# JoeHEZHAO/Optical-Flow-Guided-Feature-Pytorch

Measured on AMD Instinct MI355X. Metric: OFF-forward clips/sec (7-seg 224x224), higher is better.
Workload: dtype f32 (split-fp32: every fp32 operand as three bf16 planes = the fp32 value exactly, six exact plane products on the bf16 MFMA pipe, f32 accumulate); 1 GPU; RGB_OFF forward, batch=64 clips/GPU x 7 segments, nine 224x224-geometry feature maps; global_batch=64, segments=7, parallelism=clip-shard x1, slice_mode=reference_flat

## Files before the change

### include/offk.h

```cpp
#ifndef OFFK_H_
#define OFFK_H_

#include <stddef.h>
#include <stdint.h>

#ifdef __cplusplus
extern "C" {
#endif

#define OFFK_ABI_VERSION 10
#define OFFK_NUM_SITES 9

enum offk_status {
  OFFK_OK = 0,
  OFFK_ERR_INVALID = -1,
  OFFK_ERR_HIP = -2,
  OFFK_ERR_MISSING_WEIGHT = -3,
  OFFK_ERR_UNKNOWN_KEY = -4,
  OFFK_ERR_NO_DEVICE = -5
};

enum offk_variant {
  OFFK_VARIANT_RGB_LEARNED_DW = 0,
  OFFK_VARIANT_DIAG_SOBEL = 1
};
enum offk_slice_mode {
  OFFK_SLICE_REFERENCE_FLAT = 0,
  OFFK_SLICE_PER_CLIP = 1
};
enum offk_consensus {
  OFFK_CONSENSUS_NONE = 0,
  OFFK_CONSENSUS_AVG = 1
};
enum offk_feat_layout {
  OFFK_FEAT_NCHW = 0,
  OFFK_FEAT_NHWC = 1
};

enum offk_precision {
  OFFK_PRECISION_FP32 = 0,
  OFFK_PRECISION_F32SPLIT = 2
};

typedef struct offk_config {
  int32_t batch;
  int32_t length;
  int32_t variant;
  int32_t slice_mode;
  int32_t consensus;
  int32_t num_classes;
  int32_t feat_layout;
  int32_t device;
  int32_t precision;
} offk_config;

typedef struct offk_handle offk_handle;

int offk_abi_version(void);

const char* offk_last_error(const offk_handle* h);

int offk_create(const offk_config* cfg, offk_handle** out);
int offk_destroy(offk_handle* h);

int offk_set_weight(offk_handle* h, const char* key, const float* data, const int64_t* shape, int ndim);
int offk_bind_weight(offk_handle* h, const char* key, const float* device_data, const int64_t* shape, int ndim);
int offk_missing_weights(const offk_handle* h, char* buf, size_t buflen);

size_t offk_workspace_bytes(const offk_handle* h);

int offk_forward(offk_handle* h, void* stream, const float* const feats[OFFK_NUM_SITES],
                 float* out7, float* out14, float* out28, void* workspace);

typedef struct offk_feat_parts {
  int32_t n_parts;
  int32_t channels[4];
  const float* data[4];
} offk_feat_parts;
int offk_forward_parts(offk_handle* h, void* stream, const offk_feat_parts parts[OFFK_NUM_SITES],
                       float* out7, float* out14, float* out28, void* workspace);

enum offk_feat_dtype { OFFK_FEAT_F32 = 0, OFFK_FEAT_BF16 = 1, OFFK_FEAT_F16 = 2 };
int offk_forward_typed(offk_handle* h, void* stream, int feat_dtype, const void* const feats[OFFK_NUM_SITES],
                       float* out7, float* out14, float* out28, void* workspace);
int offk_forward_parts_typed(offk_handle* h, void* stream, int feat_dtype, const offk_feat_parts parts[OFFK_NUM_SITES],
                             float* out7, float* out14, float* out28, void* workspace);

int offk_forward_cl(offk_handle* h, void* stream, int feat_dtype, const void* const feats[OFFK_NUM_SITES],
                    float* out7, float* out14, float* out28, void* workspace);
int offk_forward_parts_cl(offk_handle* h, void* stream, int feat_dtype, const offk_feat_parts parts[OFFK_NUM_SITES],
                          float* out7, float* out14, float* out28, void* workspace);

int offk_workspace_region(const offk_handle* h, const char* name, size_t* offset_bytes, size_t* nbytes);

#define OFFK_NUM_STAGES 6
int offk_set_profiling(offk_handle* h, int enable);
int offk_stage_times(offk_handle* h, double ms[OFFK_NUM_STAGES], int64_t calls[OFFK_NUM_STAGES], int reset);
int offk_launch_times(offk_handle* h, char* names, size_t names_len, double* ms, int64_t* calls, int max_entries, int reset);


int offk_pw_reduce(offk_handle* h, void* stream, int site, const float* feat, float* G, float* D);

int offk_sobel_tdiff(offk_handle* h, void* stream, int site, const float* G, const float* D,
                     float* M, int m_cstride, int m_coff, int algo);

int offk_sobel_tdiff_all(offk_handle* h, void* stream, void* workspace, int algo);

int offk_off_units(offk_handle* h, void* stream, const float* const feats[OFFK_NUM_SITES], void* workspace);
int offk_off_units_fused(offk_handle* h, void* stream, const float* const feats[OFFK_NUM_SITES], void* workspace);
int offk_off_units_fused_typed(offk_handle* h, void* stream, int feat_dtype, const void* const feats[OFFK_NUM_SITES],
                               void* workspace);
int offk_off_units_fused_cl(offk_handle* h, void* stream, int feat_dtype, const void* const feats[OFFK_NUM_SITES],
                            void* workspace);

enum offk_conv_flags { OFFK_CONV_RELU_IN = 1, OFFK_CONV_RELU_PRE = 2, OFFK_CONV_RELU_POST = 4,
                        };
int offk_conv2d(void* stream, const float* x, int x_cstride, int x_coff, int n_img, int H, int W, int Ci,
                const float* w, const float* bias, int Co, int KH, int KW, int stride, int pad,
                const float* res, int res_cstride, int res_coff, int flags,
                float* y, int y_cstride, int y_coff);
int offk_conv2d_ex(void* stream, const float* x, int x_cstride, int x_coff, int n_img, int H, int W, int Ci,
                   const float* w, const float* bias, int Co, int KH, int KW, int stride, int pad,
                   const float* res, int res_cstride, int res_coff, int flags,
                   float* y, int y_cstride, int y_coff, int tile_cfg, int splitk, float* partial, size_t partial_floats,
                   int precision);
int offk_pack_conv_weight(void* stream, const float* w_oihw, int Co, int Ci, int KH, int KW, float* w_packed);
int offk_set_conv_plan(offk_handle* h, const char* conv_key, int tile_cfg, int splitk);

int offk_bottleneck_chain14(void* stream, const float* x, int x_cstride, int x_coff, int n_img, int Cin, int relu_in,
                            const float* w1, const float* b1, const float* w2_packed, const float* b2,
                            const float* w3, const float* b3, int K3,
                            const float* res, int res_cstride, int res_coff, float* y, int y_cstride, int y_coff);
int offk_bottleneck_chain14_split(void* stream, const float* x, int x_cstride, int x_coff, int n_img, int Cin, int relu_in,
                                  const float* w1, const float* b1, const float* w2_packed, const float* b2,
                                  const float* w3, const float* b3, const float* branch_w, const float* branch_b,
                                  const float* res, int res_cstride, int res_coff, float* y, int y_cstride, int y_coff,
                                  void* scratch, size_t scratch_bytes);
int offk_winograd_conv3x3(void* stream, const float* x, int x_cstride, int x_coff, int n_img, int Ci,
                          const float* w_packed, const float* bias, int Co,
                          const float* res, int res_cstride, int res_coff, int flags,
                          float* y, int y_cstride, int y_coff, float* scratch, size_t scratch_floats, float* pool_part);

int offk_winograd_conv5x5s2(void* stream, const float* x, int x_cstride, int x_coff, int n_img, int Ci,
                            const float* w_packed, const float* bias, int Co,
                            const float* res, int res_cstride, int res_coff, int flags,
                            float* y, int y_cstride, int y_coff, float* scratch, size_t scratch_floats);

int offk_winograd_conv7x7s2(void* stream, const float* x, int x_cstride, int x_coff, int n_img, int Ci,
                            const float* w_packed, const float* bias, int Co, int flags,
                            float* y, int y_cstride, int y_coff, float* scratch, size_t scratch_floats);

int offk_winograd_between(void* stream, const float* M, const float* bias_in, int phases_in, int n_img, int Cin,
                          float* x, int x_cstride, int x_coff, const float* w1, const float* b1, int Cmid, float* V);
int offk_winograd_between_ex(void* stream, const float* M, const float* bias_in, int phases_in, int n_img, int Cin, float* x,
                             int x_cstride, int x_coff, const float* w1, const float* b1, int Cmid, float* V, int precision,
                             void* scratch, size_t scratch_bytes);

int offk_batched_gemm_nt(void* stream, const float* x, const float* w, float* y, int batch, int M, int K, int Co, int precision,
                         void* scratch, size_t scratch_bytes);

int offk_head(void* stream, const float* x, int x_cstride, int x_coff, int n_img, int H, int W, int C,
              int maxpool, const float* fc_w, const float* fc_b, int num_classes, float* out);

int offk_segment_consensus(void* stream, const float* x, int B, int T, int C, float* out);

int offk_score_fusion(void* stream, const float* const* scores, const float* weights, int n_sets, int videos,
                      int crops, int classes, float* fused, int32_t* pred);

typedef struct offk_grad_view {
  const float* data;
  int32_t cstride;
  int32_t coff;
} offk_grad_view;

size_t offk_train_workspace_bytes(const offk_handle* h);

// ... 38 lines not shown
```

### optical-flow-guided-feature-pytorch_amd/_lib.py

```python
import ctypes
import os

HERE = os.path.dirname(os.path.abspath(__file__))
LIB_PATH = os.environ.get("OFFK_LIB") or os.path.join(HERE, "liboffk.so")
NUM_SITES = 9
NUM_STAGES = 6
STAGE_NAMES = ("pw_reduce", "sobel_tdiff", "fusion_28", "fusion_14", "fusion_7", "heads")

CONV_RELU_IN, CONV_RELU_PRE, CONV_RELU_POST = 1, 2, 4
PRECISION_FP32, PRECISION_F32SPLIT = 0, 2
PRECISIONS = {"fp32": 0, "f32split": 2}
FEAT_F32, FEAT_BF16, FEAT_F16 = 0, 1, 2


class OffkError(RuntimeError):
    pass


class OffkConfig(ctypes.Structure):
    _fields_ = [("batch", ctypes.c_int32), ("length", ctypes.c_int32), ("variant", ctypes.c_int32),
                ("slice_mode", ctypes.c_int32), ("consensus", ctypes.c_int32),
                ("num_classes", ctypes.c_int32), ("feat_layout", ctypes.c_int32),
                ("device", ctypes.c_int32), ("precision", ctypes.c_int32)]


class OffkFeatParts(ctypes.Structure):
    _fields_ = [("n_parts", ctypes.c_int32), ("channels", ctypes.c_int32 * 4), ("data", ctypes.c_void_p * 4)]


class OffkGradView(ctypes.Structure):
    _fields_ = [("data", ctypes.c_void_p), ("cstride", ctypes.c_int32), ("coff", ctypes.c_int32)]


_c = ctypes
_P = ctypes.c_void_p
_F = ctypes.c_void_p
_I = ctypes.c_int

SIGNATURES = {
    "offk_abi_version": (_I, []),
    "offk_last_error": (_c.c_char_p, [_P]),
    "offk_create": (_I, [_c.POINTER(OffkConfig), _c.POINTER(_P)]),
    "offk_destroy": (_I, [_P]),
    "offk_set_weight": (_I, [_P, _c.c_char_p, _F, _c.POINTER(_c.c_int64), _I]),
    "offk_bind_weight": (_I, [_P, _c.c_char_p, _F, _c.POINTER(_c.c_int64), _I]),
    "offk_missing_weights": (_I, [_P, _c.c_char_p, _c.c_size_t]),
    "offk_workspace_bytes": (_c.c_size_t, [_P]),
    "offk_forward": (_I, [_P, _P, _c.POINTER(_F), _F, _F, _F, _P]),
    "offk_forward_parts": (_I, [_P, _P, _c.POINTER(OffkFeatParts), _F, _F, _F, _P]),
    "offk_forward_typed": (_I, [_P, _P, _I, _c.POINTER(_P), _F, _F, _F, _P]),
    "offk_forward_parts_typed": (_I, [_P, _P, _I, _c.POINTER(OffkFeatParts), _F, _F, _F, _P]),
    "offk_forward_cl": (_I, [_P, _P, _I, _c.POINTER(_P), _F, _F, _F, _P]),
    "offk_forward_parts_cl": (_I, [_P, _P, _I, _c.POINTER(OffkFeatParts), _F, _F, _F, _P]),
    "offk_workspace_region": (_I, [_P, _c.c_char_p, _c.POINTER(_c.c_size_t), _c.POINTER(_c.c_size_t)]),
    "offk_set_profiling": (_I, [_P, _I]),
    "offk_stage_times": (_I, [_P, _c.POINTER(_c.c_double), _c.POINTER(_c.c_int64), _I]),
    "offk_launch_times": (_I, [_P, _c.c_char_p, _c.c_size_t, _c.POINTER(_c.c_double), _c.POINTER(_c.c_int64), _I, _I]),
    "offk_pw_reduce": (_I, [_P, _P, _I, _F, _F, _F]),
    "offk_sobel_tdiff": (_I, [_P, _P, _I, _F, _F, _F, _I, _I, _I]),
    "offk_sobel_tdiff_all": (_I, [_P, _P, _P, _I]),
    "offk_off_units": (_I, [_P, _P, _c.POINTER(_F), _P]),
    "offk_off_units_fused": (_I, [_P, _P, _c.POINTER(_F), _P]),
    "offk_off_units_fused_typed": (_I, [_P, _P, _I, _c.POINTER(_P), _P]),
    "offk_off_units_fused_cl": (_I, [_P, _P, _I, _c.POINTER(_P), _P]),
    "offk_conv2d": (_I, [_P, _F, _I, _I, _I, _I, _I, _I, _F, _F, _I, _I, _I, _I, _I, _F, _I, _I, _I, _F, _I, _I]),
    "offk_conv2d_ex": (_I, [_P, _F, _I, _I, _I, _I, _I, _I, _F, _F, _I, _I, _I, _I, _I, _F, _I, _I, _I, _F, _I, _I,
                            _I, _I, _F, _c.c_size_t, _I]),
    "offk_bottleneck_chain14": (_I, [_P, _F, _I, _I, _I, _I, _I, _F, _F, _F, _F, _F, _F, _I, _F, _I, _I, _F, _I, _I]),
    "offk_bottleneck_chain14_split": (_I, [_P, _F, _I, _I, _I, _I, _I, _F, _F, _F, _F, _F, _F, _F, _F, _F, _I, _I, _F, _I, _I, _P, ctypes.c_size_t]),
    "offk_winograd_conv3x3": (_I, [_P, _F, _I, _I, _I, _I, _F, _F, _I, _F, _I, _I, _I, _F, _I, _I, _F, _c.c_size_t, _F]),
    "offk_winograd_conv5x5s2": (_I, [_P, _F, _I, _I, _I, _I, _F, _F, _I, _F, _I, _I, _I, _F, _I, _I, _F, _c.c_size_t]),
    "offk_winograd_conv7x7s2": (_I, [_P, _F, _I, _I, _I, _I, _F, _F, _I, _I, _F, _I, _I, _F, _c.c_size_t]),
    "offk_winograd_between": (_I, [_P, _F, _F, _I, _I, _I, _F, _I, _I, _F, _F, _I, _F]),
    "offk_winograd_between_ex": (_I, [_P, _F, _F, _I, _I, _I, _F, _I, _I, _F, _F, _I, _F, _I, _P, ctypes.c_size_t]),
    "offk_batched_gemm_nt": (_I, [_P, _F, _F, _F, _I, _I, _I, _I, _I, _P, _c.c_size_t]),
    "offk_pack_conv_weight": (_I, [_P, _F, _I, _I, _I, _I, _F]),
    "offk_set_conv_plan": (_I, [_P, _c.c_char_p, _I, _I]),
    "offk_head": (_I, [_P, _F, _I, _I, _I, _I, _I, _I, _I, _F, _F, _I, _F]),
    "offk_segment_consensus": (_I, [_P, _F, _I, _I, _I, _F]),
    "offk_score_fusion": (_I, [_P, _c.POINTER(_F), _c.POINTER(_c.c_float), _I, _I, _I, _I, _F, _F]),
    "offk_train_workspace_bytes": (_c.c_size_t, [_P]),
    "offk_off_units_train": (_I, [_P, _P, _c.POINTER(_F), _P, _c.c_uint64, _c.c_double]),
    "offk_unit_grad_floats": (_c.c_size_t, [_P]),
    "offk_unit_grad_slot": (_I, [_P, _c.c_char_p, _c.POINTER(_c.c_size_t), _c.POINTER(_c.c_size_t)]),
    "offk_off_units_backward": (_I, [_P, _P, _c.POINTER(_F), _c.POINTER(OffkGradView), _P, _c.c_uint64, _c.c_double, _F, _I]),
    "offk_pw_reduce_typed": (_I, [_P, _P, _I, _I, _P, _F, _F]),
    "offk_off_units_typed": (_I, [_P, _P, _I, _c.POINTER(_P), _P]),
    "offk_off_units_train_typed": (_I, [_P, _P, _I, _c.POINTER(_P), _P, _c.c_uint64, _c.c_double]),
    "offk_off_units_backward_typed": (_I, [_P, _P, _I, _c.POINTER(_P), _c.POINTER(OffkGradView), _P, _c.c_uint64, _c.c_double, _F, _I]),
    "offk_pw_reduce_cl": (_I, [_P, _P, _I, _I, _P, _F, _F]),
    "offk_off_units_cl": (_I, [_P, _P, _I, _c.POINTER(_P), _P]),
    "offk_off_units_train_cl": (_I, [_P, _P, _I, _c.POINTER(_P), _P, _c.c_uint64, _c.c_double]),
    "offk_off_units_backward_cl": (_I, [_P, _P, _I, _c.POINTER(_P), _c.POINTER(OffkGradView), _P, _c.c_uint64, _c.c_double, _F, _I]),
    "offk_segment_consensus_backward": (_I, [_P, _F, _I, _I, _I, _F]),
    "offk_nchw_to_nhwc": (_I, [_P, _F, _I, _I, _I, _F]),
    "offk_nhwc_to_nchw": (_I, [_P, _F, _I, _I, _I, _I, _I, _F]),
}

_lib = None


def load():
    global _lib
    if _lib is not None:
        return _lib
    import torch
    if not os.path.exists(LIB_PATH):
        raise OffkError("liboffk.so not built: run `python -c 'import __graft_entry__ as g; g.build()'` "
                        "(or optical-flow-guided-feature-pytorch_amd/build.py); there is no fallback path")
    lib = ctypes.CDLL(LIB_PATH)
    for name, (res, args) in SIGNATURES.items():
        fn = getattr(lib, name)
        fn.restype = res
        fn.argtypes = args
    if lib.offk_abi_version() != 10:
        raise OffkError("liboffk.so ABI version mismatch")
    _lib = lib
    return lib


def check(rc, handle=None):
    if rc != 0:
        msg = load().offk_last_error(handle)
        raise OffkError("liboffk error %d: %s" % (rc, msg.decode() if msg else "?"))
```

### optical-flow-guided-feature-pytorch_amd/csrc/heads.hip

```cpp
#include "offk_common.h"
#include "offk_internal.h"

#include <mutex>
#include <set>
#include <utility>

namespace offk {

hipError_t lds_attr_once(const void* kernel, int bytes) {
  static std::mutex mu;
  static std::set<std::pair<const void*, int>> done;
  int dev = 0;
  hipError_t e = hipGetDevice(&dev);
  if (e != hipSuccess) return e;
  std::lock_guard<std::mutex> lock(mu);
  if (done.count({kernel, dev})) return hipSuccess;
  e = hipFuncSetAttribute(kernel, hipFuncAttributeMaxDynamicSharedMemorySize, bytes);
  if (e == hipSuccess) done.insert({kernel, dev});
  return e;
}

constexpr int HEAD_MAX_C = 1024;

__device__ __forceinline__ float4 add4(float4 a, float4 b) { return make_float4(a.x + b.x, a.y + b.y, a.z + b.z, a.w + b.w); }
// ... 209 lines not shown
  float pw[4];
#pragma unroll
  for (int j = 0; j < 4; ++j) {
    const int sl = min(s_lo + j, s_hi);
    const int slot = (sl * 32) / hw == img ? 0 : 1;
    ps[j] = tiles ? part + ((size_t)img * 4 + j) * C + 4 * kq : part + ((size_t)sl * 2 + slot) * C + 4 * kq;
    pw[j] = tiles || s_lo + j <= s_hi ? 1.f : 0.f;
  }
  const int per = ((C / kFcWaves + 63) / 64) * 64;
  const int kbeg = wave * per, kend = min(C, kbeg + per);
  const float* w0 = fw + (size_t)min(cls0 + li, ncls - 1) * C + 4 * kq;
  const float* w1 = fw + (size_t)min(cls0 + 16 + li, ncls - 1) * C + 4 * kq;
  fcx4 acc0 = {0.f, 0.f, 0.f, 0.f}, acc1 = {0.f, 0.f, 0.f, 0.f};
  for (int kb = kbeg; kb < kend; kb += 64) {
    fcx4 xr[4][4], a0[4], a1[4];
#pragma unroll
    for (int u = 0; u < 4; ++u) {
#pragma unroll
      for (int j = 0; j < 4; ++j) xr[u][j] = *reinterpret_cast<const fcx4*>(ps[j] + kb + 16 * u);
      a0[u] = *reinterpret_cast<const fcx4*>(w0 + kb + 16 * u);
      a1[u] = *reinterpret_cast<const fcx4*>(w1 + kb + 16 * u);
    }
#pragma unroll
    for (int u = 0; u < 4; ++u) {
      const fcx4 x = ((xr[u][0] * pw[0] + xr[u][1] * pw[1]) + xr[u][2] * pw[2]) + xr[u][3] * pw[3];
      acc0 = __builtin_amdgcn_mfma_f32_16x16x4f32(a0[u].x, x.x, acc0, 0, 0, 0);
      acc1 = __builtin_amdgcn_mfma_f32_16x16x4f32(a1[u].x, x.x, acc1, 0, 0, 0);
      acc0 = __builtin_amdgcn_mfma_f32_16x16x4f32(a0[u].y, x.y, acc0, 0, 0, 0);
      acc1 = __builtin_amdgcn_mfma_f32_16x16x4f32(a1[u].y, x.y, acc1, 0, 0, 0);
      acc0 = __builtin_amdgcn_mfma_f32_16x16x4f32(a0[u].z, x.z, acc0, 0, 0, 0);
      acc1 = __builtin_amdgcn_mfma_f32_16x16x4f32(a1[u].z, x.z, acc1, 0, 0, 0);
      acc0 = __builtin_amdgcn_mfma_f32_16x16x4f32(a0[u].w, x.w, acc0, 0, 0, 0);
      acc1 = __builtin_amdgcn_mfma_f32_16x16x4f32(a1[u].w, x.w, acc1, 0, 0, 0);
    }
  }
  red[wave][0][lane] = acc0;
  red[wave][1][lane] = acc1;
  __syncthreads();
  if (wave < 2) {
    fcx4 v = red[0][wave][lane];
#pragma unroll
    for (int w = 1; w < kFcWaves; ++w) v += red[w][wave][lane];
    const int gi = blockIdx.x * 16 + li, c = cls0 + 16 * wave + 4 * kq;
    const float inv = 1.f / (float)hw;
    if (gi < n_img) {
#pragma unroll
      for (int j = 0; j < 4; ++j)
        if (c + j < ncls) out[(size_t)gi * ncls + c + j] = v[j] * inv + fb[c + j];
    }
  }
}
__global__ __launch_bounds__(64 * kFcWaves) void fc_pooled_kernel(const float* __restrict__ part, int hw, int tiles, int n_img, int C,
                                                                  const float* __restrict__ fw, const float* __restrict__ fb, int ncls,
                                                                  float* __restrict__ out) {
  fc_pooled_body(part, hw, tiles, n_img, C, fw, fb, ncls, out);
}
__global__ __launch_bounds__(64 * kFcWaves) void fc_pooled_multi_kernel(FcPooledJobs j) {
  const FcPooledJob& h = j.job[blockIdx.z];
  fc_pooled_body(h.part, h.hw, h.tiles, j.n_img, h.C, h.fw, h.fb, j.ncls, h.out);
}
hipError_t fc_pooled_multi_launch(const FcPooledJobs& j, hipStream_t st) {
  if (j.njobs < 1 || j.njobs > 3 || j.n_img <= 0 || j.ncls <= 0) return hipErrorInvalidValue;
  for (int i = 0; i < j.njobs; ++i)
    if (j.job[i].C % 64 || j.job[i].hw < 32) return hipErrorInvalidValue;
  hipLaunchKernelGGL(fc_pooled_multi_kernel, dim3((j.n_img + 15) / 16, (j.ncls + 31) / 32, j.njobs), dim3(64 * kFcWaves), 0, st, j);
  return hipGetLastError();
}
hipError_t fc_pooled_launch(const float* part, int hw, int tiles, int n_img, int C, const float* fw, const float* fb, int ncls, float* out,
                            hipStream_t st) {
  if (C % 64 || hw < 32 || n_img <= 0 || ncls <= 0) return hipErrorInvalidValue;
  hipLaunchKernelGGL(fc_pooled_kernel, dim3((n_img + 15) / 16, (ncls + 31) / 32), dim3(64 * kFcWaves), 0, st, part, hw, tiles, n_img, C, fw, fb, ncls, out);
  return hipGetLastError();
}

__global__ void vec_add_kernel(const float* __restrict__ a, const float* __restrict__ b, float* __restrict__ o, int n) {
  int i = blockIdx.x * blockDim.x + threadIdx.x;
  if (i < n) o[i] = a[i] + b[i];
}
hipError_t vec_add_launch(const float* a, const float* b, float* o, int n, hipStream_t st) {
  hipLaunchKernelGGL(vec_add_kernel, dim3((n + 255) / 256), dim3(256), 0, st, a, b, o, n);
  return hipGetLastError();
}

__global__ void consensus_kernel(const float* __restrict__ x, int T, int C, float* __restrict__ out) {
  const int b = blockIdx.x;
  for (int c = threadIdx.x; c < C; c += blockDim.x) {
    float s = 0.f;
    for (int t = 0; t < T; ++t) s += x[((size_t)b * T + t) * C + c];
    out[(size_t)b * C + c] = s / (float)T;
  }
}
__global__ void consensus_multi_kernel(const float* x0, const float* x1, const float* x2, int T, int C, float* o0, float* o1, float* o2) {
  const float* const x = blockIdx.y == 0 ? x0 : blockIdx.y == 1 ? x1 : x2;
  float* const out = blockIdx.y == 0 ? o0 : blockIdx.y == 1 ? o1 : o2;
  const int b = blockIdx.x;
  for (int c = threadIdx.x; c < C; c += blockDim.x) {
    float s = 0.f;
    for (int t = 0; t < T; ++t) s += x[((size_t)b * T + t) * C + c];
    out[(size_t)b * C + c] = s / (float)T;
  }
}
hipError_t consensus_multi_launch(const float* const x[3], float* const out[3], int nheads, int B, int T, int C, hipStream_t st) {
  if (nheads < 1 || nheads > 3) return hipErrorInvalidValue;
  hipLaunchKernelGGL(consensus_multi_kernel, dim3(B, nheads), dim3(128), 0, st, x[0], x[1], x[2], T, C, out[0], out[1], out[2]);
  return hipGetLastError();
}
hipError_t consensus_launch(const float* x, int B, int T, int C, float* out, hipStream_t st) {
  hipLaunchKernelGGL(consensus_kernel, dim3(B), dim3(128), 0, st, x, T, C, out);
  return hipGetLastError();
}

constexpr int SF_MAX_SETS = 8;
struct ScoreFusionArgs { const float* s[SF_MAX_SETS]; float w[SF_MAX_SETS]; int n, crops, classes; float* fused; int* pred; };
__global__ __launch_bounds__(256) void score_fusion_kernel(ScoreFusionArgs a) {
  __shared__ float best_v[256];
  __shared__ int best_i[256];
  const int v = blockIdx.x, tid = threadIdx.x;
  float bv = -INFINITY;
  int bi = 0x7fffffff;
  for (int c = tid; c < a.classes; c += 256) {
    float acc = 0.f;
#pragma unroll
    for (int i = 0; i < SF_MAX_SETS; ++i)
      if (i < a.n) {
        const float* p = a.s[i] + ((size_t)v * a.crops) * a.classes + c;
        float m = 0.f;
        for (int k = 0; k < a.crops; ++k) m += p[(size_t)k * a.classes];
        acc += a.w[i] * (m / (float)a.crops);
      }
    a.fused[(size_t)v * a.classes + c] = acc;
    if (acc > bv) { bv = acc; bi = c; }
  }
  if (!a.pred) return;
  best_v[tid] = bv; best_i[tid] = bi;
  __syncthreads();
  for (int s = 128; s > 0; s >>= 1) {
    if (tid < s) {
      const float ov = best_v[tid + s];
      const int oi = best_i[tid + s];
      if (ov > best_v[tid] || (ov == best_v[tid] && oi < best_i[tid])) { best_v[tid] = ov; best_i[tid] = oi; }
    }
    __syncthreads();
  }
  if (tid == 0) a.pred[v] = best_i[0];
}
hipError_t score_fusion_launch(const float* const* scores, const float* weights, int n, int videos, int crops, int classes,
                               float* fused, int* pred, hipStream_t st) {
  if (n < 1 || n > SF_MAX_SETS) return hipErrorInvalidValue;
  ScoreFusionArgs a;
  for (int i = 0; i < SF_MAX_SETS; ++i) { a.s[i] = i < n ? scores[i] : nullptr; a.w[i] = i < n ? weights[i] : 0.f; }
  a.n = n; a.crops = crops; a.classes = classes; a.fused = fused; a.pred = pred;
  hipLaunchKernelGGL(score_fusion_kernel, dim3(videos), dim3(256), 0, st, a);
  return hipGetLastError();
}

__global__ __launch_bounds__(256) void nchw_to_nhwc_kernel(const float* __restrict__ src, int C, int HW, float* __restrict__ dst) {
  __shared__ float t[32][33];
  const int n = blockIdx.z, c0 = blockIdx.y * 32, q0 = blockIdx.x * 32;
  const int tx = threadIdx.x & 31, ty = threadIdx.x >> 5;
  for (int r = ty; r < 32; r += 8) {
    int c = c0 + r, q = q0 + tx;
    t[r][tx] = (c < C && q < HW) ? src[((size_t)n * C + c) * HW + q] : 0.f;
  }
  __syncthreads();
  for (int r = ty; r < 32; r += 8) {
    int q = q0 + r, c = c0 + tx;
// ... 32 lines not shown
```

### optical-flow-guided-feature-pytorch_amd/csrc/offk_api.hip

```cpp
#include "../../include/offk.h"

#include <algorithm>
#include <cmath>
#include <cstdio>
#include <cstdlib>
#include <cstring>
#include <map>
#include <string>
#include <vector>

#include "offk_internal.h"

using namespace offk;

typedef const void* const* MapPtrs;

static bool path_switch(const char* name, int* min_p = nullptr) {
  const char* e = getenv(name);
  if (e && min_p && atoi(e) > 1) *min_p = atoi(e);
  return !(e && *e == '0');
}

static ConvDesc conv_desc(const float* x, int x_cs, int x_coff, int n_img, int H, int W, int Ci, const float* w, const float* bias, int Co, int KH,
                          int KW, int stride, int pad, const float* res, int res_cs, int res_coff, int flags, float* y, int y_cs, int y_coff,
// ... 17 lines not shown
      a.g_x[gi] = grp[gi].v_off; a.g_w[gi] = grp[gi].u_off; a.g_y[gi] = grp[gi].m_off;
    }
    a.w_planes = U_planes;
    if (U_planes && wino_gemm_split_supported(a)) return wino_gemm_split_launch(a, s);
    if (persistent && wino_gemm_supported(a)) return wino_gemm_launch(a, s);
  }
  const int K0 = grp[0].kmul * Ci;
  ConvDesc d = conv_desc(V, K0, 0, rows, 1, 1, K0, U, nullptr, Co, 1, 1, 1, 0, nullptr, 0, 0, 0, M, Co, 0, 3, 1);
#ifdef OFFK_TUNING_KNOBS
  { const char* e = getenv("OFFK_WINO_CFG"); if (e && (Co % 128 == 0 || atoi(e) == 1 || atoi(e) == 2)) d.tile_cfg = atoi(e); }
#endif
  d.batch = npoints; d.x_bstride = (long long)rows * K0; d.w_bstride = (long long)Co * K0; d.y_bstride = (long long)rows * Co;
  if (ngrp > 1) {
    d.ngroups = ngrp;
    for (int gi = 0; gi < ngrp; ++gi) {
      d.g_batch[gi] = grp[gi].batch; d.g_Ci[gi] = grp[gi].kmul * Ci;
      d.g_x[gi] = grp[gi].v_off; d.g_w[gi] = grp[gi].u_off; d.g_y[gi] = grp[gi].m_off;
    }
  }
  return conv2d_launch(d, s, why);
}
static bool wino_gemm_stage_default() {
  static const bool on = path_switch("OFFK_WINO_GEMM");
  return on;
}

namespace {

struct SiteSpec { const char* name; int C, H; };
const SiteSpec kSites[kNumSites] = {{"3a", 256, 28}, {"3b", 320, 28}, {"3c", 576, 14}, {"4a", 576, 14}, {"4b", 576, 14},
                                    {"4c", 608, 14}, {"4d", 608, 14}, {"5a", 1024, 7}, {"5b", 1024, 7}};
const int kPwOrder[kNumSites] = {7, 8, 5, 6, 2, 3, 4, 1, 0};
const int kSiteFusion[kNumSites] = {0, 0, 1, 1, 1, 1, 1, 2, 2};
const int kSiteCoff[kNumSites] = {0, 160, 0, 160, 320, 480, 640, 0, 160};
const int kFusionC[3] = {320, 1056, 832};

struct ConvSpec { const char* key; int Co, Ci, K, stride, pad; };
enum ConvId {
  C_T28, C1_28A, C2_28A, C3_28A, CB_28A, C1_28B, C2_28B, C3_28B, C1_28C, C2_28C, C3_28C,
  C_T14, C1_14A, C2_14A, C3_14A, CE_14A, C1_14B, C2_14B, C3_14B,
  C_T7, C1_7, C2_7, C3_7, CB_7, kNumConvs
};
const ConvSpec kConvs[kNumConvs] = {
    {"motion_conv_trans_28", 64, 320, 7, 2, 3},      {"motion_conv1_trans_28a", 64, 64, 1, 1, 0},
    {"motion_conv2_trans_28a", 64, 64, 3, 1, 1},     {"motion_conv3_trans_28a", 256, 64, 1, 1, 0},
    {"motion_conv_branch_28a", 256, 64, 1, 1, 0},    {"motion_conv1_trans_28b", 64, 256, 1, 1, 0},
    {"motion_conv2_trans_28b", 64, 64, 3, 1, 1},     {"motion_conv3_trans_28b", 256, 64, 1, 1, 0},
    {"motion_conv1_trans_28c", 64, 256, 1, 1, 0},    {"motion_conv2_trans_28c", 64, 64, 3, 1, 1},
    {"motion_conv3_trans_28c", 256, 64, 1, 1, 0},    {"motion_conv_trans_14", 128, 1056, 5, 2, 2},
    {"motion_conv1_trans_14a", 128, 128, 1, 1, 0},   {"motion_conv2_trans_14a", 128, 128, 3, 1, 1},
    {"motion_conv3_trans_14a", 512, 128, 1, 1, 0},   {"motion_conv_expand_trans_14a", 512, 128, 1, 1, 0},
    {"motion_conv1_trans_14b", 128, 512, 1, 1, 0},   {"motion_conv2_trans_14b", 128, 128, 3, 1, 1},
    {"motion_conv3_trans_14b", 512, 128, 3, 1, 1},   {"motion_conv_trans", 256, 832, 3, 1, 1},
    {"motion_conv1_trans", 256, 256, 1, 1, 0},       {"motion_conv2_trans", 256, 256, 3, 1, 1},
    {"motion_conv3_trans", 1024, 256, 1, 1, 0},      {"motion_conv_branch_trans", 1024, 256, 1, 1, 0}};
struct MergedSpec { const char* name; int main_id, branch_id; };
const MergedSpec kMerged[3] = {{"merged_28a", C3_28A, CB_28A}, {"merged_14a", C3_14A, CE_14A}, {"merged_7", C3_7, CB_7}};
const int kTunedP240[kNumConvs][2] = {
    {3, 2}, {-1, 0}, {-1, 0}, {-1, 0}, {-1, 0}, {-1, 0}, {-1, 0}, {-1, 0}, {-1, 0}, {-1, 0}, {-1, 0},
    {4, 4}, {-1, 0}, {-1, 0}, {-1, 0}, {-1, 0}, {-1, 0}, {-1, 0}, {-1, 0},
    {-1, 0}, {-1, 0}, {-1, 0}, {-1, 0}, {-1, 0}};
const int kMergedPlan[2][3][2] = {
    {{3, 1}, {3, 1}, {3, 1}},
    {{1, 1}, {3, 1}, {3, 1}}};
struct HeadSpec { const char* key; int C; };
const HeadSpec kHeads[3] = {{"fc_action_motion", 1024}, {"fc_action_motion_28", 256}, {"fc_action_motion_14", 512}};
const char* kSobelKey = "sobel_edge_diagonal.conv.weight";

enum SlotKind { SK_GEN_W, SK_GEN_B, SK_DOWN_W, SK_DOWN_B, SK_DW_W, SK_DW_B, SK_SOBEL, SK_CONV_W, SK_CONV_B, SK_FC_W, SK_FC_B };
struct Slot {
  std::string key;
  std::vector<int64_t> shape;
  SlotKind kind;
  int idx;
  bool set = false;
};

struct Derived {
  float* u = nullptr;
  float* u_planes = nullptr;
  float* u2 = nullptr;
  float* planes = nullptr;
  float* gemm_planes = nullptr;
};
constexpr int kNumDerived = kNumConvs + 3;
constexpr int merged_slot(int m) { return kNumConvs + m; }

thread_local std::string g_err;

size_t align_up(size_t v, size_t a) { return (v + a - 1) / a * a; }

}

struct offk_handle {
  offk_config cfg;
  int N = 0, P = 0;
  std::vector<Slot> slots;
  std::map<std::string, int> index;
  float* pw_w[kNumSites] = {};
  float* pw_wt16[kNumSites] = {};
  float* pw_wt16s[kNumSites] = {};
  bool split_gemm = false;
  int split_gemm_skip = 0;
  bool split_chain = false;
  bool split_mid = false;
  bool f32split = false;
  bool pw_dirty = true;
  float* pw_b[kNumSites] = {};
  float* dw_w[kNumSites] = {};
  float* dw_b[kNumSites] = {};
  const float* bnd_gen_w[kNumSites] = {};
  const float* bnd_gen_b[kNumSites] = {};
  const float* bnd_down_w[kNumSites] = {};
  const float* bnd_down_b[kNumSites] = {};
  const float* bnd_dw_w[kNumSites] = {};
  const float* bnd_dw_b[kNumSites] = {};
  float* sobel_w = nullptr;
  bool sobel_taps4 = false;
  float* conv_w[kNumConvs] = {};
  float* conv_b[kNumConvs] = {};
  float* fc_w[3] = {};
  float* fc_b[3] = {};
  float* merged_w[3] = {};
  float* merged_b[3] = {};
  int merged_cfg[3] = {3, 3, 3}, merged_sk[3] = {1, 1, 1};
  bool merged_dirty = true;

  float* zero_page = nullptr;
  bool fused_units = true;
  bool winograd = true;
  bool wino_7x7 = true;
  int wino7_min_p = 12;
  Derived derived[kNumDerived];
  bool derived_dirty = true;
  bool chain_wino = false;
  int wino5_min_p = 40;
  bool wino_5x5 = true;
  bool wino_gemm = true;
  bool wino_mid = true;
  bool chain = true;
  int chain_min_p = 72;
  size_t train_ws_bytes = 0;
  int wg_kpb = 0;
  std::map<std::string, std::pair<size_t, size_t>> grad_slots;
  size_t grad_floats = 0;

  int conv_cfg[kNumConvs];
  int conv_splitk[kNumConvs];
  size_t splitk_floats = 0;
  bool fold_pool = true;
  std::vector<void*> allocs;
  std::map<std::string, std::pair<size_t, size_t>> regions;
  size_t ws_bytes = 0;
  int profiling = 0;
  std::vector<hipEvent_t> events;
  size_t ev_used = 0;
  std::vector<hipEvent_t> tr_events;
  std::vector<int> tr_marks;
  std::vector<std::string> tr_names;
  mutable std::string err;
};

namespace {

int fail(offk_handle* h, int code, const std::string& msg) {
  if (h) h->err = msg;
  g_err = msg;
  return code;
}
int fail_hip(offk_handle* h, hipError_t e, const char* what) {
  return fail(h, OFFK_ERR_HIP, std::string(what) + ": " + hipGetErrorString(e));
}
#define HIP_TRY(h, expr)                                   \
  do {                                                     \
    hipError_t e__ = (expr);                               \
    if (e__ != hipSuccess) return fail_hip(h, e__, #expr); \
  } while (0)
#define TRY(expr)            \
  do {                       \
    int rc__ = (expr);       \
    if (rc__ != OFFK_OK) return rc__; \
  } while (0)

constexpr size_t kTraceMaxEvents = 1 << 16;
int trace_mark(offk_handle* h, hipStream_t st, const char* name) {
  if (h->profiling != 2 || h->tr_marks.size() >= kTraceMaxEvents) return OFFK_OK;
  int id = -1;
  if (name) {
    for (size_t i = 0; i < h->tr_names.size() && id < 0; ++i)
      if (h->tr_names[i] == name) id = (int)i;
    if (id < 0) { id = (int)h->tr_names.size(); h->tr_names.push_back(name); }
  }
  if (h->tr_marks.size() >= h->tr_events.size()) {
    hipEvent_t e;
    HIP_TRY(h, hipEventCreate(&e));
    h->tr_events.push_back(e);
  }
  HIP_TRY(h, hipEventRecord(h->tr_events[h->tr_marks.size()], st));
  h->tr_marks.push_back(id);
  return OFFK_OK;
}

int dev_alloc(offk_handle* h, float** p, size_t nfloats) {
  void* q = nullptr;
  HIP_TRY(h, hipMalloc(&q, nfloats * sizeof(float)));
  HIP_TRY(h, hipMemset(q, 0, nfloats * sizeof(float)));
  h->allocs.push_back(q);
  *p = static_cast<float*>(q);
  return OFFK_OK;
}

void add_slot(offk_handle* h, const std::string& key, std::vector<int64_t> shape, SlotKind kind, int idx) {
  Slot s;
  s.key = key; s.shape = std::move(shape); s.kind = kind; s.idx = idx;
  h->index[key] = (int)h->slots.size();
  h->slots.push_back(std::move(s));
}

void add_region(offk_handle* h, const std::string& name, size_t nfloats) {
  size_t off = align_up(h->ws_bytes, 256);
  h->regions[name] = std::make_pair(off, nfloats * sizeof(float));
  h->ws_bytes = off + nfloats * sizeof(float);
}

float* region(const offk_handle* h, void* ws, const char* name) {
  auto it = h->regions.find(name);
  return reinterpret_cast<float*>(static_cast<char*>(ws) + it->second.first);
}

void ub_plan(int H, int* strips, int* rows) {
  *rows = H >= 28 ? 7 : H;
  *strips = (H + *rows - 1) / *rows;
}
constexpr int kUbTpix = 8;

void plan_workspace(offk_handle* h) {
  const size_t N = h->N, P = h->P;
  for (int s = 0; s < kNumSites; ++s) {
    size_t hw = (size_t)kSites[s].H * kSites[s].H;
    add_region(h, std::string("G_") + kSites[s].name, N * hw * kGenCh);
    add_region(h, std::string("D_") + kSites[s].name, P * hw * kDownCh);
  }
  add_region(h, "fusion_28", P * 784 * 320);
  add_region(h, "fusion_14", P * 196 * 1056);
  add_region(h, "fusion_7", P * 49 * 832);
  add_region(h, "xt_28", P * 196 * 128);
  add_region(h, "t1_28", P * 196 * 64);
  add_region(h, "sa_28", P * 196 * 256);
  add_region(h, "sb_28", P * 196 * 256);
  add_region(h, "xu_14", P * 49 * 256);
  add_region(h, "u1_14", P * 49 * 128);
  add_region(h, "sa_14", P * 49 * 512);
  add_region(h, "xv_7", P * 49 * 512);
  add_region(h, "v1_7", P * 49 * 256);
  add_region(h, "sum_7", P * 49 * 1024);
  add_region(h, "logit_7", P * (size_t)h->cfg.num_classes);
  add_region(h, "logit_14", P * (size_t)h->cfg.num_classes);
  add_region(h, "logit_28", P * (size_t)h->cfg.num_classes);
  add_region(h, "pooled_7", P * 1024);
  add_region(h, "pooled_14", P * 512);
  add_region(h, "pooled_28", P * 256);
  add_region(h, "poolpart_28", (size_t)4 * P * 256);
  add_region(h, "poolpart_7", ((P * 49 + 31) / 32) * 2 * 1024);
  add_region(h, "poolpart_14", ((P * 49 + 31) / 32) * 2 * 512);
  if (h->cfg.precision == OFFK_PRECISION_FP32) {
    add_region(h, "wino_v", std::max((size_t)kWinoUnits4 * P * 1056, (size_t)kWino7Tiles * P * kWino7Units * 320));
    add_region(h, "wino_m", (size_t)kWinoPoints * P * 512);
    add_region(h, "poolpart_14t", (size_t)4 * P * 512);
  }
  h->splitk_floats = (size_t)std::min<size_t>(64, std::max<size_t>(8, 1536 / P)) * P * 196 * 64;
  add_region(h, "splitk", h->splitk_floats);
  h->ws_bytes = align_up(h->ws_bytes, 256);

  const size_t fwd_bytes = h->ws_bytes;
  long long work = 0;
  for (int s = 0; s < kNumSites; ++s) {
    const int hw = kSites[s].H * kSites[s].H;
    work += (long long)N * ((hw + 31) / 32) * ((kSites[s].C + 127) / 128);
  }
  h->wg_kpb = (int)std::max<long long>(4, (work + 1535) / 1536);
  for (int s = 0; s < kNumSites; ++s) {
    const size_t hw = (size_t)kSites[s].H * kSites[s].H;
    const std::string n = kSites[s].name;
    int strips, rows;
    ub_plan(kSites[s].H, &strips, &rows);
    const size_t kt_total = N * ((hw + 31) / 32), nchunks = (kt_total + h->wg_kpb - 1) / h->wg_kpb;
    const size_t cpad = (size_t)((kSites[s].C + 127) / 128) * 128;
    add_region(h, "dG_" + n, N * hw * kGenCh);
    add_region(h, "dD_" + n, P * hw * kDownCh);
    add_region(h, "dwp_" + n, P * strips * 10 * kDownCh);
    add_region(h, "wgs_" + n, nchunks * kUnitCh * cpad);
    add_region(h, "wgb_" + n, nchunks * kUnitCh);
    auto slot = [&](const std::string& key, size_t count) {
      h->grad_slots[key] = std::make_pair(h->grad_floats, count);
      h->grad_floats += count;
    };
    slot("motion_conv_gen_" + n + ".weight", (size_t)kGenCh * kSites[s].C);
    slot("motion_conv_gen_" + n + ".bias", kGenCh);
    slot("motion_spatial_down_" + n + ".weight", (size_t)kDownCh * kSites[s].C);
    slot("motion_spatial_down_" + n + ".bias", kDownCh);
    if (h->cfg.variant != OFFK_VARIANT_DIAG_SOBEL) {
      slot("motion_spatial_grad_" + n + ".weight", (size_t)kDownCh * 9);
      slot("motion_spatial_grad_" + n + ".bias", kDownCh);
    }
  }
  h->train_ws_bytes = align_up(h->ws_bytes, 256);
  h->ws_bytes = fwd_bytes;
}

struct DeviceGuard {
  int prev = -1;
  bool changed = false;
  explicit DeviceGuard(int want) {
    if (hipGetDevice(&prev) == hipSuccess && prev != want) changed = hipSetDevice(want) == hipSuccess;
  }
  ~DeviceGuard() { if (changed) (void)hipSetDevice(prev); }
};

int check_ready(offk_handle* h) {
  for (const Slot& s : h->slots)
    if (!s.set) return fail(h, OFFK_ERR_MISSING_WEIGHT, "weight not set: " + s.key);
  return OFFK_OK;
}

bool slot_set(const offk_handle* h, const std::string& key) {
  auto it = h->index.find(key);
  return it != h->index.end() && h->slots[it->second].set;
}

int site_weights_ready(offk_handle* h, int site, bool need_pw, bool need_dw) {
  const std::string n = kSites[site].name;
  if (need_pw)
    for (const char* k : {"motion_conv_gen_", "motion_spatial_down_"})
      for (const char* sfx : {".weight", ".bias"})
        if (!slot_set(h, std::string(k) + n + sfx)) return fail(h, OFFK_ERR_MISSING_WEIGHT, std::string("weight not set: ") + k + n + sfx);
  if (need_dw) {
    if (h->cfg.variant == OFFK_VARIANT_DIAG_SOBEL) {
      if (!slot_set(h, kSobelKey)) return fail(h, OFFK_ERR_MISSING_WEIGHT, std::string("weight not set: ") + kSobelKey);
    } else {
      for (const char* sfx : {".weight", ".bias"})
        if (!slot_set(h, "motion_spatial_grad_" + n + sfx)) return fail(h, OFFK_ERR_MISSING_WEIGHT, "weight not set: motion_spatial_grad_" + n + sfx);
    }
  }
  return OFFK_OK;
}

void pw_weight_ptrs(const offk_handle* h, int site, const float** w, const float** w_down, const float** b,
                    const float** b_down) {
  const float* own = h->pw_w[site];
  *w = h->bnd_gen_w[site] ? h->bnd_gen_w[site] : own;
  *w_down = h->bnd_down_w[site] ? h->bnd_down_w[site] : own + (size_t)kGenCh * kSites[site].C;
// ... 177 lines not shown
  pt.f32split = h->f32split;
  for (int s = 0; s < kNumSites; ++s)
    if (h->bnd_gen_w[s] || h->bnd_down_w[s]) pt.bdirect = 0;
  const char* fus[3] = {"fusion_28", "fusion_14", "fusion_7"};
  for (int i = 0; i < kNumSites; ++i) {
    const int s = kPwOrder[i];
    PtSite& o = pt.s[i];
    const offk_feat_parts& fp = feats[s];
    for (int q = 0; q < 4; ++q) { o.xp[q] = q < fp.n_parts ? fp.data[q] : nullptr; o.cp[q] = q < fp.n_parts ? fp.channels[q] : 0; }
    o.nparts = fp.n_parts;
    pw_weight_ptrs(h, s, &o.w, &o.w_down, &o.bias, &o.bias_down);
    o.wt = nullptr;
    o.wt16 = h->pw_wt16[s];
    o.wt16s = h->pw_wt16s[s];
    o.D = region(h, ws, (std::string("D_") + kSites[s].name).c_str());
    o.M = region(h, ws, fus[kSiteFusion[s]]);
    o.m_cs = kFusionC[kSiteFusion[s]]; o.m_coff = kSiteCoff[s];
    o.C = kSites[s].C; o.HW = kSites[s].H * kSites[s].H;
  }
  if (ev) HIP_TRY(h, hipEventRecord(ev[0], st));
  TRY(launch_k1t(h, st, pt, feat_dtype, cl));
  if (ev) HIP_TRY(h, hipEventRecord(ev[1], st));
  { int rc = trace_mark(h, st, "units:sobel S-blocks (K2 spatial half)"); if (rc != OFFK_OK) return rc; }
  { int rc = run_sobel_tdiff_all(h, st, ws, 3); if (rc != OFFK_OK) return rc; }
  if (ev) HIP_TRY(h, hipEventRecord(ev[2], st));
  return OFFK_OK;
}

int check_feat_train(offk_handle* h, const FeatKind& k, int feat_dtype, const void* const* feats, int first, int count, const char* fn) {
  const std::string f(fn), maps = std::string(": ") + k.noun + " feature map";
  if (!(feat_dtype == OFFK_FEAT_F32 && k.f32_ok) && feat_dtype != OFFK_FEAT_BF16 && feat_dtype != OFFK_FEAT_F16)
    return fail(h, OFFK_ERR_INVALID, f + ": unknown feat_dtype " + std::to_string(feat_dtype) + " (OFFK_FEAT_F32 / _BF16 / _F16)");
  if (!k.cl && h->cfg.feat_layout == OFFK_FEAT_NHWC) return fail(h, OFFK_ERR_INVALID, f + maps + "s are NCHW-only (this handle is NHWC)");
  for (int i = 0; i < count; ++i) {
    const SiteSpec& site = kSites[first + i];
    if (!feats[i]) return fail(h, OFFK_ERR_INVALID, f + ": null feature map");
    if (reinterpret_cast<uintptr_t>(feats[i]) & (k.align_train - 1))
      return fail(h, OFFK_ERR_INVALID, f + maps + " pointers must be " + std::to_string(k.align_train) + "-byte aligned (site " + site.name + ")");
    if (feat_dtype != OFFK_FEAT_F32 && (unsigned long long)h->N * site.H * site.H * site.C * 2ull >= kFeat16MaxBytes)
      return fail(h, OFFK_ERR_INVALID, f + ": 16-bit feature maps of 2 GiB or more are not supported (site " + site.name + ")");
  }
  return OFFK_OK;
}

int pw_reduce_site(offk_handle* h, void* stream, const FeatKind* k, int feat_dtype, int site, const void* feat, float* G, float* D, const char* fn) {
  if (!h || site < 0 || site >= kNumSites || !feat || !G || !D) return fail(h, OFFK_ERR_INVALID, std::string(fn) + ": bad argument");
  if (k) TRY(check_feat_train(h, *k, feat_dtype, &feat, site, 1, fn));
  TRY(site_weights_ready(h, site, true, false));
  DeviceGuard guard(h->cfg.device);
  hipStream_t st = static_cast<hipStream_t>(stream);
  PwParams pp;
  memset(&pp, 0, sizeof(pp));
  pp.nsites = 1; pp.L = h->cfg.length; pp.P = h->P; pp.slice_mode = h->cfg.slice_mode;
  pp.nhwc = k ? k->cl : h->cfg.feat_layout == OFFK_FEAT_NHWC;
  pp.zeros = h->zero_page;
  TRY(finalize_pw(h, st));
  fill_pw_site(h, site, whole_map(site, static_cast<const float*>(feat)), G, D, &pp.s[0]);
  pp.total_blocks = pw_blocks_for(pp.s[0].M);
  return launch_k1(h, st, pp, feat_dtype, false);
}

int off_units_whole(offk_handle* h, void* stream, const FeatKind* k, int feat_dtype, const void* const feats[OFFK_NUM_SITES], void* workspace,
                    bool train, uint64_t drop_seed, double drop_p, const char* fn) {
  if (!h || !feats || !workspace) return fail(h, OFFK_ERR_INVALID, std::string(fn) + ": null argument");
  DropCfg drop;
  if (train) TRY(make_drop(h, drop_seed, drop_p, &drop));
  if (k) TRY(check_feat_train(h, *k, feat_dtype, feats, 0, kNumSites, fn));
  offk_feat_parts parts[kNumSites];
  TRY(whole_maps(h, feats, parts, fn));
  for (int s = 0; s < kNumSites; ++s) TRY(site_weights_ready(h, s, true, true));
  DeviceGuard guard(h->cfg.device);
  return run_off_units(h, static_cast<hipStream_t>(stream), parts, workspace, nullptr, k ? k->cl : h->cfg.feat_layout == OFFK_FEAT_NHWC, drop,
                       feat_dtype);
}

struct View { const float* p; int cs, coff; };

enum DerivedKind {
  DK_U_F43,
  DK_U_POLY,
  DK_U_F54,
  DK_CHAIN_U2,
  DK_PLANES,
  DK_U_PLANES
};
DerivedKind u_kind(const ConvSpec& c) { return c.K == 7 ? DK_U_F54 : c.K == 5 ? DK_U_POLY : DK_U_F43; }
int u_units(DerivedKind k) { return k == DK_U_F54 ? kWino7Units : k == DK_U_POLY ? kWinoUnits4 : kWinoPoints; }
size_t u_elems(const ConvSpec& c) { return (size_t)u_units(u_kind(c)) * c.Co * c.Ci; }
int wino_phases(const ConvSpec& c) { return u_kind(c) == DK_U_POLY ? 4 : 1; }
int wino_conv_groups(const ConvSpec& c, long long rows, WinoGroup grp[4]) {
  return u_kind(c) == DK_U_F54 ? wino7_groups(rows, c.Ci, c.Co, grp) : wino_groups(wino_phases(c), rows, c.Ci, c.Co, grp);
}
size_t plane_floats(size_t elems) { return (elems * 3 + 1) / 2; }

enum { ON_7X7 = 1, ON_SPLIT_GEMM = 2, ON_CHAIN_WINO = 4, ON_SPLIT_CHAIN = 8, ON_SPLIT_MID = 16 };
struct DerivedRow {
  int slot;
  DerivedKind kind;
  float* Derived::*image;
  int needs = 0;
  int skip_bit = 0;
  int alloc_K = 0;
};
bool derived_exists(const offk_handle* h, const DerivedRow& r) {
  const int on = h->wino_7x7 * ON_7X7 | h->split_gemm * ON_SPLIT_GEMM | h->chain_wino * ON_CHAIN_WINO | (h->chain && h->split_chain) * ON_SPLIT_CHAIN |
                 (h->wino_mid && h->split_mid) * ON_SPLIT_MID;
  const bool shape = r.kind != DK_U_PLANES || (kConvs[r.slot].Co % 64 == 0 && kConvs[r.slot].Ci >= 64);
  return h->winograd && !(r.needs & ~on) && shape && !(h->split_gemm_skip & r.skip_bit);
}

const DerivedRow kDerived[] = {
    {C3_14B, DK_U_F43, &Derived::u}, {C_T7, DK_U_F43, &Derived::u}, {C2_7, DK_U_F43, &Derived::u}, {C2_14A, DK_U_F43, &Derived::u},
    {C2_14B, DK_U_F43, &Derived::u}, {C_T14, DK_U_POLY, &Derived::u}, {C_T28, DK_U_F54, &Derived::u, ON_7X7},
    {C3_14B, DK_U_PLANES, &Derived::u_planes, ON_SPLIT_GEMM, 1}, {C_T7, DK_U_PLANES, &Derived::u_planes, ON_SPLIT_GEMM, 2},
    {C2_7, DK_U_PLANES, &Derived::u_planes, ON_SPLIT_GEMM, 4}, {C2_14A, DK_U_PLANES, &Derived::u_planes, ON_SPLIT_GEMM, 8},
    {C2_14B, DK_U_PLANES, &Derived::u_planes, ON_SPLIT_GEMM, 16}, {C_T14, DK_U_PLANES, &Derived::u_planes, ON_SPLIT_GEMM, 32},
    {C_T28, DK_U_PLANES, &Derived::u_planes, ON_7X7 | ON_SPLIT_GEMM, 64},
    {merged_slot(1), DK_PLANES, &Derived::gemm_planes, ON_SPLIT_GEMM, 128}, {merged_slot(2), DK_PLANES, &Derived::gemm_planes, ON_SPLIT_GEMM, 128},
    {C1_14B, DK_PLANES, &Derived::gemm_planes, ON_SPLIT_GEMM, 128},
    {C2_28A, DK_CHAIN_U2, &Derived::u2, ON_CHAIN_WINO}, {C2_28B, DK_CHAIN_U2, &Derived::u2, ON_CHAIN_WINO}, {C2_28C, DK_CHAIN_U2, &Derived::u2, ON_CHAIN_WINO},
    {C1_28A, DK_PLANES, &Derived::planes, ON_SPLIT_CHAIN, 0, 256}, {C2_28A, DK_PLANES, &Derived::planes, ON_SPLIT_CHAIN}, {C3_28A, DK_PLANES, &Derived::planes, ON_SPLIT_CHAIN},
    {CB_28A, DK_PLANES, &Derived::planes, ON_SPLIT_CHAIN},
    {C1_28B, DK_PLANES, &Derived::planes, ON_SPLIT_CHAIN}, {C2_28B, DK_PLANES, &Derived::planes, ON_SPLIT_CHAIN}, {C3_28B, DK_PLANES, &Derived::planes, ON_SPLIT_CHAIN},
    {C1_28C, DK_PLANES, &Derived::planes, ON_SPLIT_CHAIN}, {C2_28C, DK_PLANES, &Derived::planes, ON_SPLIT_CHAIN}, {C3_28C, DK_PLANES, &Derived::planes, ON_SPLIT_CHAIN},
    {C1_14A, DK_PLANES, &Derived::planes, ON_SPLIT_MID}, {C1_7, DK_PLANES, &Derived::planes, ON_SPLIT_MID}};

struct Matrix { const float* w; int Co, K; };
Matrix slot_matrix(const offk_handle* h, int slot) {
  if (slot < kNumConvs) return Matrix{h->conv_w[slot], kConvs[slot].Co, kConvs[slot].Ci * kConvs[slot].K * kConvs[slot].K};
  const MergedSpec& m = kMerged[slot - kNumConvs];
  return Matrix{h->merged_w[slot - kNumConvs], kConvs[m.main_id].Co, kConvs[m.main_id].Ci + kConvs[m.branch_id].Ci};
}
size_t derived_floats(const offk_handle* h, const DerivedRow& r) {
  switch (r.kind) {
    case DK_U_F43: case DK_U_POLY: case DK_U_F54: return (size_t)u_units(r.kind) * kConvs[r.slot].Co * kConvs[r.slot].Ci;
    case DK_CHAIN_U2: return (size_t)16 * 64 * 64;
    case DK_PLANES: { const Matrix m = slot_matrix(h, r.slot); return plane_floats((size_t)m.Co * (r.alloc_K ? r.alloc_K : m.K)); }
    case DK_U_PLANES: return plane_floats(u_elems(kConvs[r.slot]));
  }
  return 0;
}
int pack_derived(offk_handle* h, const DerivedRow& r, hipStream_t st) {
  const Derived& d = h->derived[r.slot];
  switch (r.kind) {
    case DK_U_F43: case DK_U_POLY:
      HIP_TRY(h, wino_weight_launch(h->conv_w[r.slot], kConvs[r.slot].Co, kConvs[r.slot].Ci, wino_phases(kConvs[r.slot]), d.u, st));
      break;
    case DK_U_F54: HIP_TRY(h, wino7_weight_launch(h->conv_w[r.slot], kConvs[r.slot].Co, kConvs[r.slot].Ci, d.u, st)); break;
    case DK_CHAIN_U2: HIP_TRY(h, chain_wino_weight_launch(h->conv_w[r.slot], d.u2, st)); break;
    case DK_PLANES: {
      const Matrix m = slot_matrix(h, r.slot);
      HIP_TRY(h, wino_pack_split_launch(m.w, d.*r.image, m.Co, m.K, 1, st));
      break;
    }
    case DK_U_PLANES: {
      const ConvSpec& c = kConvs[r.slot];
      WinoGroup grp[4];
      const int ngrp = wino_conv_groups(c, 1, grp);
      for (int g = 0; g < ngrp; ++g)
        HIP_TRY(h, wino_pack_split_launch(d.u + grp[g].u_off, reinterpret_cast<char*>(d.u_planes) + grp[g].u_off * 6, c.Co, grp[g].kmul * c.Ci, grp[g].batch, st));
      break;
    }
  }
  return OFFK_OK;
}

int finalize_merged(offk_handle* h, hipStream_t st) {
  if (!h->merged_dirty) return OFFK_OK;
  for (int m = 0; m < 3; ++m) {
    const ConvSpec& a = kConvs[kMerged[m].main_id];
    const ConvSpec& b = kConvs[kMerged[m].branch_id];
    const size_t K = (size_t)a.Ci + b.Ci;
    HIP_TRY(h, hipMemcpy2DAsync(h->merged_w[m], K * 4, h->conv_w[kMerged[m].main_id], (size_t)a.Ci * 4, (size_t)a.Ci * 4, a.Co, hipMemcpyDeviceToDevice, st));
    HIP_TRY(h, hipMemcpy2DAsync(h->merged_w[m] + a.Ci, K * 4, h->conv_w[kMerged[m].branch_id], (size_t)b.Ci * 4, (size_t)b.Ci * 4, a.Co, hipMemcpyDeviceToDevice, st));
    HIP_TRY(h, vec_add_launch(h->conv_b[kMerged[m].main_id], h->conv_b[kMerged[m].branch_id], h->merged_b[m], a.Co, st));
  }
  h->merged_dirty = false;
  return OFFK_OK;
}
int finalize_derived(offk_handle* h, hipStream_t st) {
  if (!h->derived_dirty) return OFFK_OK;
  for (const DerivedRow& r : kDerived)
    if (h->derived[r.slot].*r.image) TRY(pack_derived(h, r, st));
  h->derived_dirty = false;
  return OFFK_OK;
}

constexpr int RI = OFFK_CONV_RELU_IN_, RP = OFFK_CONV_RELU_PRE_, RO = OFFK_CONV_RELU_POST_;
int trace_mark(offk_handle* h, hipStream_t st, const char* key, const char* what) {
  return h->profiling != 2 ? OFFK_OK : trace_mark(h, st, (std::string(key) + what).c_str());
}
WinoMidArgs wino_mid_args(const float* M, const float* bias_in, int phases_in, int n_img, int Cin, float* x, int x_cs, int x_coff, const float* w1,
                          const float* b1, int Cmid, float* V, const void* w1p = nullptr) {
  WinoMidArgs m;
  m.M = M; m.bias_in = bias_in; m.phases_in = phases_in; m.x = x; m.x_cs = x_cs; m.x_coff = x_coff;
  m.w1 = w1; m.b1 = b1; m.Cin = Cin; m.Cmid = Cmid; m.n_img = n_img; m.V = V; m.w1p = w1p;
  return m;
}
ChainArgs chain_args(const float* x, int x_cs, int x_coff, int n_img, int Cin, int relu_in, const float* w1, const float* b1, const float* w2,
                     const float* b2, const float* w3, const float* b3, int K3, const float* res, int res_cs, int res_coff, float* y, int y_cs,
                     int y_coff) {
  ChainArgs a{};
  a.x = x; a.x_cs = x_cs; a.x_coff = x_coff; a.Cin = Cin; a.relu_in = relu_in ? 1 : 0;
  a.w1 = w1; a.b1 = b1; a.w2 = w2; a.b2 = b2; a.w3 = w3; a.b3 = b3; a.K3 = K3;
  a.res = res; a.res_cs = res_cs; a.res_coff = res_coff; a.y = y; a.y_cs = y_cs; a.y_coff = y_coff;
  a.n_img = n_img; a.relu_out = 1;
  const unsigned long long xb = ((unsigned long long)n_img * 196 * x_cs - x_coff) * 4ull;
  a.x_bytes = xb < 0x7fffffffull ? (unsigned)xb : 0u;
  return a;
}

struct Fwd {
  offk_handle* h;
  hipStream_t s;
  void* ws;
  int n;
  hipEvent_t* ev = nullptr;
  float *F14, *F7;
  float *wino_V, *wino_M;
  float* splitk;
  float *out7, *out14, *out28;
  float *l7, *l14, *l28;
  FcPooledJobs fcj{};
  bool wino, w7, mid, w5, chained, fold, fold14t;

  float* reg(const char* name) const { return region(h, ws, name); }

  int init(offk_handle* handle, hipStream_t st, void* workspace, float* o7, float* o14, float* o28) {
    h = handle; s = st; ws = workspace; n = h->P; out7 = o7; out14 = o14; out28 = o28;
    if (h->profiling == 1) {
      const size_t per = OFFK_NUM_STAGES + 1;
      if ((h->ev_used + 1) * per > h->events.size() && h->events.size() < 4096 * per) {
        for (size_t i = 0; i < per; ++i) {
          hipEvent_t e;
          HIP_TRY(h, hipEventCreate(&e));
          h->events.push_back(e);
        }
      }
      if ((h->ev_used + 1) * per <= h->events.size()) ev = &h->events[h->ev_used++ * per];
    }
    wino = h->winograd;
    w7 = h->derived[C_T28].u && wino && h->wino_7x7 && n >= h->wino7_min_p;
    mid = wino && h->wino_mid;
    w5 = wino && h->wino_5x5 && n >= h->wino5_min_p;
    chained = h->chain && n >= h->chain_min_p && (unsigned long long)n * 196 * 256 * 4ull < 0x7fffffffull;
    auto generic = [](int cfg) { return cfg != 6 && cfg != 7 && cfg != 10; };
    fold = h->fold_pool && generic(h->conv_cfg[C3_14B]) && generic(h->merged_cfg[2]);
    fold14t = wino && h->fold_pool;
    F14 = reg("fusion_14"); F7 = reg("fusion_7"); splitk = reg("splitk");
    wino_V = wino ? reg("wino_v") : nullptr;
    wino_M = wino ? reg("wino_m") : nullptr;
    const bool cons = h->cfg.consensus == OFFK_CONSENSUS_AVG;
    l7 = cons ? reg("logit_7") : out7; l14 = cons ? reg("logit_14") : out14; l28 = cons ? reg("logit_28") : out28;
    fcj.n_img = n; fcj.ncls = h->cfg.num_classes;
    return OFFK_OK;
  }

  int conv_raw(const char* name, int Co, int Ci, int K, int stride, int pad, const float* w, const float* bias, int cfg, int sk, int H, View x,
               const float* res, int res_cs, int res_coff, int flags, float* y, int y_cs, int y_coff, const void* w_planes, float* pool_part) {
    if (w_planes && K == 1 && stride == 1 && pad == 0 && !res && !(flags & OFFK_CONV_RELU_IN_)) {
      WinoGemmArgs a{};
      a.x = x.p; a.w = w; a.y = y; a.M = n * H * H; a.Co = Co; a.ngroups = 1; a.g_batch[0] = 1; a.g_K[0] = Ci;
      a.w_planes = w_planes;
      a.epilogue = 1; a.x_rs = x.cs; a.x_coff = x.coff; a.y_rs = y_cs; a.y_coff = y_coff; a.bias = bias;
      a.relu = (flags & (OFFK_CONV_RELU_PRE_ | OFFK_CONV_RELU_POST_)) ? 1 : 0;
      a.pool_part = pool_part; a.pool_hw = pool_part ? H * H : 0;
      if (wino_gemm_split_supported(a)) {
        TRY(trace_mark(h, s, name));
        hipError_t e = wino_gemm_split_launch(a, s);
        if (e != hipSuccess) return fail_hip(h, e, name);
        return OFFK_OK;
      }
    }
    ConvDesc d = conv_desc(x.p, x.cs, x.coff, n, H, H, Ci, w, bias, Co, K, K, stride, pad, res, res_cs, res_coff, flags, y, y_cs, y_coff, cfg, sk,
                           splitk, h->splitk_floats, h->cfg.precision);
    d.pool_part = pool_part; d.pool_hw = pool_part ? H * H / (stride * stride) : 0;
    const char* why = nullptr;
    TRY(trace_mark(h, s, name));
    hipError_t e = conv2d_launch(d, s, &why);
    if (e != hipSuccess) return fail(h, why ? OFFK_ERR_INVALID : OFFK_ERR_HIP, std::string(name) + ": " + (why ? why : hipGetErrorString(e)));
    return OFFK_OK;
  }
  int conv(ConvId id, int H, View x, const float* res, int res_cs, int res_coff, int flags, float* y, int y_cs, int y_coff, float* pool_part = nullptr) {
    const ConvSpec& c = kConvs[id];
    return conv_raw(c.key, c.Co, c.Ci, c.K, c.stride, c.pad, h->conv_w[id], h->conv_b[id], h->conv_cfg[id], h->conv_splitk[id], H, x, res, res_cs,
                    res_coff, flags, y, y_cs, y_coff, h->derived[id].gemm_planes, pool_part);
  }
  int conv_merged(int m, int H, View x, int flags, float* y, int y_cs, int y_coff, float* pool_part = nullptr) {
    const Matrix w = slot_matrix(h, merged_slot(m));
    return conv_raw(kMerged[m].name, w.Co, w.K, 1, 1, 0, w.w, h->merged_b[m], h->merged_cfg[m], h->merged_sk[m], H, x, nullptr, 0, 0, flags, y, y_cs,
                    y_coff, h->derived[merged_slot(m)].gemm_planes, pool_part);
  }

  int wino_in(ConvId id, View x) {
    const ConvSpec& c = kConvs[id];
    TRY(trace_mark(h, s, c.key, " [winograd: input transform]"));
    if (u_kind(c) == DK_U_F54) HIP_TRY(h, wino7_input_launch(x.p, x.cs, x.coff, n, c.Ci, wino_V, s));
    else HIP_TRY(h, wino_input_launch(x.p, x.cs, x.coff, n, c.Ci, wino_phases(c), wino_V, s));
    return OFFK_OK;
  }
  int wino_mm(ConvId id) {
    const ConvSpec& c = kConvs[id];
    const bool f54 = u_kind(c) == DK_U_F54;
    TRY(trace_mark(h, s, c.key, f54 ? " [winograd: 64 GEMMs]" : " [winograd: 121 GEMMs]"));
    const int rows = f54 ? kWino7Tiles * n : n;
    WinoGroup grp[4];
    const int ngrp = wino_conv_groups(c, rows, grp);
    const char* why = nullptr;
    hipError_t e = wino_gemms_launch(grp, ngrp, f54 ? kWino7Points : kWinoPoints, rows, c.Ci, c.Co, wino_V, h->derived[id].u, wino_M, h->wino_gemm, s, &why,
                                     h->derived[id].u_planes);
    if (e != hipSuccess) return fail(h, why ? OFFK_ERR_INVALID : OFFK_ERR_HIP, std::string(c.key) + " (winograd): " + (why ? why : hipGetErrorString(e)));
    return OFFK_OK;
  }
  int wino_out(ConvId id, const float* res, int res_cs, int res_coff, int flags, float* y, int y_cs, int y_coff, float* pool_t) {
    const ConvSpec& c = kConvs[id];
    TRY(trace_mark(h, s, c.key, " [winograd: output transform]"));
    if (u_kind(c) == DK_U_F54) HIP_TRY(h, wino7_output_launch(wino_M, n, c.Co, h->conv_b[id], flags, y, y_cs, y_coff, s));
    else HIP_TRY(h, wino_output_launch(wino_M, n, c.Co, wino_phases(c), h->conv_b[id], res, res_cs, res_coff, flags, y, y_cs, y_coff, pool_t, s));
    return OFFK_OK;
  }
  int wino_conv(ConvId id, View x, const float* res, int res_cs, int res_coff, int flags, float* y, int y_cs, int y_coff, float* pool_t) {
    TRY(wino_in(id, x));
    TRY(wino_mm(id));
    return wino_out(id, res, res_cs, res_coff, flags, y, y_cs, y_coff, pool_t);
  }
  int wino_between(ConvId a, ConvId c1, float* xa, int xa_cs, int xa_coff, const char* name) {
    const bool has = c1 != kNumConvs;
    const WinoMidArgs m = wino_mid_args(wino_M, h->conv_b[a], wino_phases(kConvs[a]), n, kConvs[a].Co, xa, xa_cs, xa_coff, has ? h->conv_w[c1] : nullptr,
                                        has ? h->conv_b[c1] : nullptr, kConvs[has ? c1 : a].Co, wino_V, has ? h->derived[c1].planes : nullptr);
    TRY(trace_mark(h, s, name));
    HIP_TRY(h, wino_mid_launch(m, s));
    return OFFK_OK;
  }
  int conv_t_c1_c2(ConvId ct, bool wino_t, int H, View F, ConvId c1, ConvId c2, float* xx, int cs, float* t, const char* between) {
    const int half = cs / 2;
    if (wino_t && mid) {
      TRY(wino_in(ct, F));
      TRY(wino_mm(ct));
      TRY(wino_between(ct, c1, xx, cs, half, between));
      TRY(wino_mm(c2));
      return wino_out(c2, nullptr, 0, 0, RP, xx, cs, 0, nullptr);
    }
    if (wino_t) TRY(wino_conv(ct, F, nullptr, 0, 0, RP, xx, cs, half, nullptr));
    else TRY(conv(ct, H, F, nullptr, 0, 0, RP, xx, cs, half));
    TRY(conv(c1, 7, View{xx, cs, half}, nullptr, 0, 0, RP, t, half, 0));
    if (wino) return wino_conv(c2, View{t, half, 0}, nullptr, 0, 0, RP, xx, cs, 0, nullptr);
    return conv(c2, 7, View{t, half, 0}, nullptr, 0, 0, RP, xx, cs, 0);
  }

  int chain(const char* name, View x, int Cin, int relu_in, ConvId c1, ConvId c2, ConvId c3, int m, bool split_branch, const float* res, float* y, int y_cs, int y_coff) {
    const bool merged = m >= 0 && !split_branch;
    ChainArgs a = chain_args(x.p, x.cs, x.coff, n, Cin, relu_in, h->conv_w[c1], h->conv_b[c1], h->conv_w[c2], h->conv_b[c2],
                             merged ? h->merged_w[m] : h->conv_w[c3], merged ? h->merged_b[m] : h->conv_b[c3], merged ? 128 : 64, res, 256, 0, y, y_cs, y_coff);
    a.u2 = h->derived[c2].u2;
    a.w1p = h->derived[c1].planes; a.w2p = h->derived[c2].planes; a.w3p = h->derived[c3].planes;
    if (split_branch) { a.wbp = h->derived[kMerged[m].branch_id].planes; a.bbr = h->conv_b[kMerged[m].branch_id]; }
    TRY(trace_mark(h, s, name));
    const char* why = nullptr;
    hipError_t e = chain14_split_supported(a) ? chain14_split_launch(a, s, &why) : chain14_launch(a, s, &why);
    if (e != hipSuccess) return fail(h, why ? OFFK_ERR_INVALID : OFFK_ERR_HIP, std::string(name) + ": " + (why ? why : hipGetErrorString(e)));
    return OFFK_OK;
  }

  int head(int k, float* logits, const float* part, int tiles, const float* x, int x_cs, int x_coff, int Hh, int maxpool, const char* pooled_name) {
    const int C = kHeads[k].C;
    if (part) { fcj.job[fcj.njobs++] = FcPooledJob{part, 49, tiles, C, h->fc_w[k], h->fc_b[k], logits}; return OFFK_OK; }
    float* pooled = reg(pooled_name);
    TRY(trace_mark(h, s, k == 0 ? "head_7 (pool + fc)" : k == 1 ? "head_28 (pool + fc)" : "head_14 (pool + fc)"));
    hipError_t e = pool_launch(x, x_cs, x_coff, n, Hh, Hh, C, maxpool, pooled, s);
    if (e == hipSuccess) e = fc_launch(pooled, n, C, h->fc_w[k], h->fc_b[k], h->cfg.num_classes, logits, s);
    if (e != hipSuccess) return fail_hip(h, e, "head");
    return OFFK_OK;
  }

  int units(const offk_feat_parts feats[], int feat_dtype, bool cl) {
    if (cl) return run_off_units_fused(h, s, feats, ws, ev, feat_dtype, true);
    if (h->fused_units && h->cfg.feat_layout != OFFK_FEAT_NHWC) return run_off_units_fused(h, s, feats, ws, ev, feat_dtype);
    return run_off_units(h, s, feats, ws, ev, h->cfg.feat_layout == OFFK_FEAT_NHWC);
  }

  int fusion28() {
    float *F28 = reg("fusion_28"), *xt = reg("xt_28"), *t1 = reg("t1_28"), *sa = reg("sa_28"), *sb = reg("sb_28");
    if (w7) TRY(wino_conv(C_T28, View{F28, 320, 0}, nullptr, 0, 0, 0, xt, 128, 64, nullptr));
    else TRY(conv(C_T28, 28, View{F28, 320, 0}, nullptr, 0, 0, 0, xt, 128, 64));
    if (chained) {
      TRY(chain("chain_28a = motion_conv1_trans_28a + motion_conv2_trans_28a + merged_28a", View{xt, 128, 64}, 64, 1, C1_28A, C2_28A, C3_28A, 0,
                h->derived[CB_28A].planes != nullptr, nullptr, sa, 256, 0));
      TRY(chain("chain_28b = motion_conv1_trans_28b + motion_conv2_trans_28b + motion_conv3_trans_28b", View{sa, 256, 0}, 256, 0, C1_28B, C2_28B, C3_28B,
                -1, false, sa, sb, 256, 0));
      TRY(chain("chain_28c = motion_conv1_trans_28c + motion_conv2_trans_28c + motion_conv3_trans_28c", View{sb, 256, 0}, 256, 0, C1_28C, C2_28C, C3_28C,
                -1, false, sb, F14, 1056, 800));
    } else {
      TRY(conv(C1_28A, 14, View{xt, 128, 64}, nullptr, 0, 0, RI | RP, t1, 64, 0));
      TRY(conv(C2_28A, 14, View{t1, 64, 0}, nullptr, 0, 0, RP, xt, 128, 0));
      TRY(conv_merged(0, 14, View{xt, 128, 0}, RO, sa, 256, 0));
      TRY(conv(C1_28B, 14, View{sa, 256, 0}, nullptr, 0, 0, RP, t1, 64, 0));
      TRY(conv(C2_28B, 14, View{t1, 64, 0}, nullptr, 0, 0, RP, xt, 128, 0));
      TRY(conv(C3_28B, 14, View{xt, 128, 0}, sa, 256, 0, RO, sb, 256, 0));
      TRY(conv(C1_28C, 14, View{sb, 256, 0}, nullptr, 0, 0, RP, t1, 64, 0));
      TRY(conv(C2_28C, 14, View{t1, 64, 0}, nullptr, 0, 0, RP, xt, 128, 0));
      TRY(conv(C3_28C, 14, View{xt, 128, 0}, sb, 256, 0, RO, F14, 1056, 800));
    }
    if (ev) HIP_TRY(h, hipEventRecord(ev[3], s));
    if (!out28) return OFFK_OK;
    float* pp = nullptr;
    if (h->fold_pool) {
      pp = reg("poolpart_28");
      TRY(trace_mark(h, s, "head_28 (max pool rows)"));
      HIP_TRY(h, maxpool_rows_launch(F14, 1056, 800, n, 14, 14, 256, pp, s));
    }
    return head(1, l28, pp, 1, F14, 1056, 800, 14, 1, "pooled_28");
  }

  int fusion14() {
    float *xu = reg("xu_14"), *u1 = reg("u1_14"), *s14 = reg("sa_14");
    TRY(conv_t_c1_c2(C_T14, w5, 14, View{F14, 1056, 0}, C1_14A, C2_14A, xu, 256, u1,
                     "motion_conv_trans_14 out + motion_conv1_trans_14a + motion_conv2_trans_14a in [winograd: between]"));
    TRY(conv_merged(1, 7, View{xu, 256, 0}, RO, s14, 512, 0));
    TRY(conv(C1_14B, 7, View{s14, 512, 0}, nullptr, 0, 0, RP, u1, 128, 0));
    float* pp14t = fold14t ? reg("poolpart_14t") : nullptr;
    float* pp14 = !wino && fold ? reg("poolpart_14") : nullptr;
    if (mid) {
      TRY(wino_in(C2_14B, View{u1, 128, 0}));
      TRY(wino_mm(C2_14B));
      TRY(wino_between(C2_14B, kNumConvs, nullptr, 0, 0, "motion_conv2_trans_14b out + motion_conv3_trans_14b in [winograd: between]"));
      TRY(wino_mm(C3_14B));
      TRY(wino_out(C3_14B, s14, 512, 0, RP | RO, F7, 832, 320, pp14t));
    } else if (wino) {
      TRY(wino_conv(C2_14B, View{u1, 128, 0}, nullptr, 0, 0, RP, xu, 256, 0, nullptr));
      TRY(wino_conv(C3_14B, View{xu, 256, 0}, s14, 512, 0, RP | RO, F7, 832, 320, pp14t));
    } else {
      TRY(conv(C2_14B, 7, View{u1, 128, 0}, nullptr, 0, 0, RP, xu, 256, 0));
      TRY(conv(C3_14B, 7, View{xu, 256, 0}, s14, 512, 0, RP | RO, F7, 832, 320, pp14));
    }
    if (ev) HIP_TRY(h, hipEventRecord(ev[4], s));
    return head(2, l14, pp14t ? pp14t : pp14, pp14t ? 1 : 0, F7, 832, 320, 7, 0, "pooled_14");
  }

  int fusion7() {
    float *xv = reg("xv_7"), *v1 = reg("v1_7"), *s7 = reg("sum_7");
    TRY(conv_t_c1_c2(C_T7, wino, 7, View{F7, 832, 0}, C1_7, C2_7, xv, 512, v1,
                     "motion_conv_trans out + motion_conv1_trans + motion_conv2_trans in [winograd: between]"));
    float* pp7 = fold ? reg("poolpart_7") : nullptr;
    TRY(conv_merged(2, 7, View{xv, 512, 0}, 0, s7, 1024, 0, pp7));
    if (ev) HIP_TRY(h, hipEventRecord(ev[5], s));
    return head(0, l7, pp7, 0, s7, 1024, 0, 7, 0, "pooled_7");
  }

  int heads() {
    if (fcj.njobs > 0) {
      TRY(trace_mark(h, s, "heads (fc on folded pools, one launch)"));
      HIP_TRY(h, fc_pooled_multi_launch(fcj, s));
    }
    if (h->cfg.consensus == OFFK_CONSENSUS_AVG) {
      TRY(trace_mark(h, s, "consensus (K6)"));
      const float* const cx[3] = {l7, l14, out28 ? l28 : l14};
      float* const co[3] = {out7, out14, out28 ? out28 : out14};
      HIP_TRY(h, consensus_multi_launch(cx, co, out28 ? 3 : 2, h->cfg.batch, h->cfg.length - 1, h->cfg.num_classes, s));
    }
    if (ev) HIP_TRY(h, hipEventRecord(ev[6], s));
    return trace_mark(h, s, nullptr);
  }
};
}

extern "C" {

int offk_abi_version(void) { return OFFK_ABI_VERSION; }

const char* offk_last_error(const offk_handle* h) { return h ? h->err.c_str() : g_err.c_str(); }

int offk_create(const offk_config* cfg, offk_handle** out) {
  if (!cfg || !out) return fail(nullptr, OFFK_ERR_INVALID, "offk_create: null argument");
  *out = nullptr;
  if (cfg->batch < 1 || cfg->length < 2) return fail(nullptr, OFFK_ERR_INVALID, "offk_create: need batch >= 1 and length >= 2");
  if (cfg->variant != OFFK_VARIANT_RGB_LEARNED_DW && cfg->variant != OFFK_VARIANT_DIAG_SOBEL) return fail(nullptr, OFFK_ERR_INVALID, "offk_create: bad variant");
  if (cfg->slice_mode != OFFK_SLICE_REFERENCE_FLAT && cfg->slice_mode != OFFK_SLICE_PER_CLIP) return fail(nullptr, OFFK_ERR_INVALID, "offk_create: bad slice_mode");
  if (cfg->consensus != OFFK_CONSENSUS_NONE && cfg->consensus != OFFK_CONSENSUS_AVG) return fail(nullptr, OFFK_ERR_INVALID, "offk_create: bad consensus");
  if (cfg->feat_layout != OFFK_FEAT_NCHW && cfg->feat_layout != OFFK_FEAT_NHWC) return fail(nullptr, OFFK_ERR_INVALID, "offk_create: bad feat_layout");
  if (cfg->precision != OFFK_PRECISION_FP32 && cfg->precision != OFFK_PRECISION_F32SPLIT)
    return fail(nullptr, OFFK_ERR_INVALID, "offk_create: bad precision (0 = fp32, 2 = f32split; 1 was the two-plane bf16x3 mode, retired in ABI v9)");
  if (cfg->num_classes < 1 || cfg->num_classes > 4096) return fail(nullptr, OFFK_ERR_INVALID, "offk_create: bad num_classes");
  if ((long long)cfg->batch * cfg->length * 784 * 320 > 0x7fffffffLL) return fail(nullptr, OFFK_ERR_INVALID, "offk_create: batch*length too large for one call; shard the clips");
  int ndev = 0;
  if (hipGetDeviceCount(&ndev) != hipSuccess || cfg->device < 0 || cfg->device >= ndev)
    return fail(nullptr, OFFK_ERR_NO_DEVICE, "offk_create: HIP device not available");
  hipDeviceProp_t prop;
  if (hipGetDeviceProperties(&prop, cfg->device) != hipSuccess || !strstr(prop.gcnArchName, "gfx950"))
    return fail(nullptr, OFFK_ERR_NO_DEVICE, "offk_create: device is not gfx950 (MI355X); this library has no other code path");

  offk_handle* h = new offk_handle();
  h->cfg = *cfg;
  offk_config cfg_in = *cfg;
  if (cfg_in.precision == OFFK_PRECISION_F32SPLIT) { h->f32split = true; h->cfg.precision = cfg_in.precision = OFFK_PRECISION_FP32; }
  cfg = &cfg_in;
  h->N = cfg->batch * cfg->length;
  h->P = cfg->batch * (cfg->length - 1);
  for (int c = 0; c < kNumConvs; ++c) {
    const int (*tab)[2] = h->P == 240 ? kTunedP240 : nullptr;
    h->conv_cfg[c] = tab ? tab[c][0] : -1;
    h->conv_splitk[c] = tab ? tab[c][1] : 0;
  }
  for (int m = 0; m < 3; ++m) {
    const int (*mp)[2] = kMergedPlan[h->P == 240];
    h->merged_cfg[m] = mp[m][0];
    h->merged_sk[m] = mp[m][1];
  }
  DeviceGuard guard(cfg->device);
  int rc = OFFK_OK;
  for (int s = 0; s < kNumSites && rc == OFFK_OK; ++s) {
    const std::string n = kSites[s].name;
    const int C = kSites[s].C;
    add_slot(h, "motion_conv_gen_" + n + ".weight", {kGenCh, C, 1, 1}, SK_GEN_W, s);
    add_slot(h, "motion_conv_gen_" + n + ".bias", {kGenCh}, SK_GEN_B, s);
    add_slot(h, "motion_spatial_down_" + n + ".weight", {kDownCh, C, 1, 1}, SK_DOWN_W, s);
    add_slot(h, "motion_spatial_down_" + n + ".bias", {kDownCh}, SK_DOWN_B, s);
    rc = dev_alloc(h, &h->pw_w[s], (size_t)kUnitCh * C);
    if (rc == OFFK_OK && cfg->precision == OFFK_PRECISION_FP32) rc = dev_alloc(h, &h->pw_wt16[s], (size_t)kUnitCh * C);
    if (rc == OFFK_OK && h->f32split) rc = dev_alloc(h, &h->pw_wt16s[s], (size_t)kUnitCh * C * 3 / 2);
    if (rc == OFFK_OK) rc = dev_alloc(h, &h->pw_b[s], kUnitCh);
    if (cfg->variant == OFFK_VARIANT_RGB_LEARNED_DW && rc == OFFK_OK) {
      add_slot(h, "motion_spatial_grad_" + n + ".weight", {kDownCh, 1, 3, 3}, SK_DW_W, s);
      add_slot(h, "motion_spatial_grad_" + n + ".bias", {kDownCh}, SK_DW_B, s);
      rc = dev_alloc(h, &h->dw_w[s], 9 * kDownCh);
      if (rc == OFFK_OK) rc = dev_alloc(h, &h->dw_b[s], kDownCh);
    }
  }
  if (cfg->variant == OFFK_VARIANT_DIAG_SOBEL && rc == OFFK_OK) {
    add_slot(h, kSobelKey, {kDownCh, 1, 3, 3}, SK_SOBEL, 0);
    rc = dev_alloc(h, &h->sobel_w, 9 * kDownCh);
  }
  for (int c = 0; c < kNumConvs && rc == OFFK_OK; ++c) {
    const ConvSpec& cs = kConvs[c];
    add_slot(h, std::string(cs.key) + ".weight", {cs.Co, cs.Ci, cs.K, cs.K}, SK_CONV_W, c);
    add_slot(h, std::string(cs.key) + ".bias", {cs.Co}, SK_CONV_B, c);
    rc = dev_alloc(h, &h->conv_w[c], (size_t)cs.Co * cs.Ci * cs.K * cs.K);
    if (rc == OFFK_OK) rc = dev_alloc(h, &h->conv_b[c], cs.Co);
  }
  for (int m = 0; m < 3 && rc == OFFK_OK; ++m) {
    const ConvSpec& a = kConvs[kMerged[m].main_id];
    const ConvSpec& b = kConvs[kMerged[m].branch_id];
    const size_t n = (size_t)a.Co * (a.Ci + b.Ci);
    rc = dev_alloc(h, &h->merged_w[m], n);
    if (rc == OFFK_OK) rc = dev_alloc(h, &h->merged_b[m], a.Co);
  }
  for (int k = 0; k < 3 && rc == OFFK_OK; ++k) {
    add_slot(h, std::string(kHeads[k].key) + ".weight", {cfg->num_classes, kHeads[k].C}, SK_FC_W, k);
    add_slot(h, std::string(kHeads[k].key) + ".bias", {cfg->num_classes}, SK_FC_B, k);
    rc = dev_alloc(h, &h->fc_w[k], (size_t)cfg->num_classes * kHeads[k].C);
    if (rc == OFFK_OK) rc = dev_alloc(h, &h->fc_b[k], cfg->num_classes);

  }
  if (rc == OFFK_OK) rc = dev_alloc(h, &h->zero_page, 64);
  h->fused_units = path_switch("OFFK_FUSED_UNITS");
  h->split_chain = h->f32split && path_switch("OFFK_SPLIT_CHAIN");
  h->split_mid = h->f32split && path_switch("OFFK_SPLIT_MID");
  {
    int from = 0;
    h->chain = path_switch("OFFK_CHAIN", &from);
    if (from) h->chain_min_p = from;
    else if (h->split_chain) h->chain_min_p = 1;
  }
  h->fold_pool = path_switch("OFFK_FOLD_POOL");
  h->wino_mid = path_switch("OFFK_WINO_MID");
  h->wino_gemm = path_switch("OFFK_WINO_GEMM");
  h->winograd = path_switch("OFFK_WINOGRAD") && cfg->precision == OFFK_PRECISION_FP32;
  h->wino_5x5 = path_switch("OFFK_WINOGRAD_5X5", &h->wino5_min_p);
  h->wino_7x7 = path_switch("OFFK_WINOGRAD_7X7", &h->wino7_min_p);
  h->split_gemm = h->winograd && h->f32split && path_switch("OFFK_SPLIT_GEMM");
#ifdef OFFK_TUNING_KNOBS
  { const char* e = getenv("OFFK_SPLIT_GEMM_SKIP"); if (e) h->split_gemm_skip = atoi(e); }
#endif
  h->chain_wino = h->winograd && h->chain && path_switch("OFFK_CHAIN_WINO");
  for (const DerivedRow& r : kDerived)
    if (rc == OFFK_OK && derived_exists(h, r)) rc = dev_alloc(h, &(h->derived[r.slot].*r.image), derived_floats(h, r));
  if (rc != OFFK_OK) {
    g_err = h->err;
    offk_destroy(h);
    return rc;
  }
  plan_workspace(h);
  *out = h;
  return OFFK_OK;
}

int offk_destroy(offk_handle* h) {
  if (!h) return OFFK_OK;
  DeviceGuard guard(h->cfg.device);
  for (hipEvent_t e : h->events) (void)hipEventDestroy(e);
  for (hipEvent_t e : h->tr_events) (void)hipEventDestroy(e);
  for (void* p : h->allocs) (void)hipFree(p);
  delete h;
  return OFFK_OK;
}

int offk_set_weight(offk_handle* h, const char* key, const float* data, const int64_t* shape, int ndim) {
  if (!h || !key || !data || !shape) return fail(h, OFFK_ERR_INVALID, "offk_set_weight: null argument");
  std::string k(key);
  if (k.compare(0, 7, "module.") == 0) k = k.substr(7);
  auto it = h->index.find(k);
  if (it == h->index.end()) return fail(h, OFFK_ERR_UNKNOWN_KEY, "offk_set_weight: not an OFF sub-network key for this variant: " + k);
  Slot& s = h->slots[it->second];
  bool ok = ndim == (int)s.shape.size();
  size_t n = 1;
  for (int i = 0; ok && i < ndim; ++i) { ok = shape[i] == s.shape[i]; n *= (size_t)s.shape[i]; }
  if (!ok) return fail(h, OFFK_ERR_INVALID, "offk_set_weight: shape mismatch for " + k);
  DeviceGuard guard(h->cfg.device);
  HIP_TRY(h, hipDeviceSynchronize());
  const size_t bytes = n * sizeof(float);
  auto copy = [&](float* dst) -> int {
    HIP_TRY(h, hipMemcpy(dst, data, bytes, hipMemcpyDefault));
    return OFFK_OK;
  };
  auto staged = [&](auto&& pack) -> int {
    void* tmp = nullptr;
    HIP_TRY(h, hipMalloc(&tmp, bytes));
    hipError_t e = hipMemcpy(tmp, data, bytes, hipMemcpyDefault);
    if (e == hipSuccess) e = pack(static_cast<const float*>(tmp));
    if (e == hipSuccess) e = hipStreamSynchronize(nullptr);
    (void)hipFree(tmp);
    if (e != hipSuccess) return fail_hip(h, e, "offk_set_weight pack");
    return OFFK_OK;
  };
  int rc = OFFK_OK;
  const int i = s.idx;
  switch (s.kind) {
    case SK_GEN_W: rc = copy(h->pw_w[i]); break;
    case SK_DOWN_W: rc = copy(h->pw_w[i] + (size_t)kGenCh * kSites[i].C); break;
    case SK_GEN_B: rc = copy(h->pw_b[i]); break;
    case SK_DOWN_B: rc = copy(h->pw_b[i] + kGenCh); break;
    case SK_DW_W: rc = staged([&](const float* t) { return repack_dw_launch(t, h->dw_w[i], nullptr); }); break;
    case SK_DW_B: rc = copy(h->dw_b[i]); break;
    case SK_SOBEL: {
      rc = staged([&](const float* t) { return repack_dw_launch(t, h->sobel_w, nullptr); });
      std::vector<float> host(n);
      if (rc == OFFK_OK && hipMemcpy(host.data(), data, bytes, hipMemcpyDefault) == hipSuccess) {
        bool four = true;
        for (int c = 0; c < kDownCh && four; ++c)
          for (int tap : {0, 2, 4, 6, 8}) four = four && host[(size_t)c * 9 + tap] == 0.f;
        h->sobel_taps4 = four;
      } else {
        h->sobel_taps4 = false;
      }
      break;
    }
    case SK_CONV_W:
      if (kConvs[i].K == 1) rc = copy(h->conv_w[i]);
      else rc = staged([&](const float* t) { return pack_conv_weight_launch(t, kConvs[i].Co, kConvs[i].Ci, kConvs[i].K, kConvs[i].K, h->conv_w[i], nullptr); });
      break;
    case SK_CONV_B: rc = copy(h->conv_b[i]); break;
    case SK_FC_W: rc = copy(h->fc_w[i]); break;
    case SK_FC_B: rc = copy(h->fc_b[i]); break;
  }
  if (rc == OFFK_OK) {
    s.set = true;
    switch (s.kind) {
      case SK_GEN_W: h->bnd_gen_w[i] = nullptr; break;
      case SK_GEN_B: h->bnd_gen_b[i] = nullptr; break;
      case SK_DOWN_W: h->bnd_down_w[i] = nullptr; break;
      case SK_DOWN_B: h->bnd_down_b[i] = nullptr; break;
      case SK_DW_W: h->bnd_dw_w[i] = nullptr; break;
      case SK_DW_B: h->bnd_dw_b[i] = nullptr; break;
      default: break;
    }
  }
  if (s.kind == SK_CONV_W || s.kind == SK_CONV_B) h->merged_dirty = true;
  if (s.kind == SK_CONV_W) h->derived_dirty = true;
  if (s.kind == SK_GEN_W || s.kind == SK_DOWN_W) h->pw_dirty = true;
  return rc;
}

int offk_bind_weight(offk_handle* h, const char* key, const float* device_data, const int64_t* shape, int ndim) {
  if (!h || !key || !device_data || !shape) return fail(h, OFFK_ERR_INVALID, "offk_bind_weight: null argument");
  std::string k(key);
  if (k.compare(0, 7, "module.") == 0) k = k.substr(7);
  auto it = h->index.find(k);
  if (it == h->index.end()) return fail(h, OFFK_ERR_UNKNOWN_KEY, "offk_bind_weight: not an OFF sub-network key for this variant: " + k);
  Slot& s = h->slots[it->second];
  bool shape_ok = ndim == (int)s.shape.size();
  size_t need = sizeof(float);
  for (int i = 0; shape_ok && i < ndim; ++i) { shape_ok = shape[i] == s.shape[i]; need *= (size_t)s.shape[i]; }
  if (!shape_ok) return fail(h, OFFK_ERR_INVALID, "offk_bind_weight: shape mismatch for " + k);
  if ((reinterpret_cast<uintptr_t>(device_data) & 15) != 0) return fail(h, OFFK_ERR_INVALID, "offk_bind_weight: pointer must be 16-byte aligned: " + k);
  hipPointerAttribute_t attr;
  if (hipPointerGetAttributes(&attr, device_data) != hipSuccess || attr.type != hipMemoryTypeDevice || attr.device != h->cfg.device) {
    (void)hipGetLastError();
    return fail(h, OFFK_ERR_INVALID, "offk_bind_weight: needs a device pointer on the handle's device: " + k);
  }
  {
    hipDeviceptr_t base = nullptr;
    size_t asz = 0;
    if (hipMemGetAddressRange(&base, &asz, const_cast<float*>(device_data)) == hipSuccess) {
      const size_t off = (size_t)(reinterpret_cast<const char*>(device_data) - reinterpret_cast<const char*>(base));
      if (off > asz || asz - off < need) return fail(h, OFFK_ERR_INVALID, "offk_bind_weight: allocation too small for " + k);
    } else {
      (void)hipGetLastError();
    }
  }
  const int i = s.idx;
  switch (s.kind) {
    case SK_GEN_W: h->bnd_gen_w[i] = device_data; break;
    case SK_GEN_B: h->bnd_gen_b[i] = device_data; break;
    case SK_DOWN_W: h->bnd_down_w[i] = device_data; break;
    case SK_DOWN_B: h->bnd_down_b[i] = device_data; break;
    case SK_DW_W: h->bnd_dw_w[i] = device_data; break;
    case SK_DW_B: h->bnd_dw_b[i] = device_data; break;
    default:
      return fail(h, OFFK_ERR_INVALID, "offk_bind_weight: only the OFF units' parameters (motion_conv_gen_*, motion_spatial_down_*, "
                                       "motion_spatial_grad_*) can be bound in place: " + k);
  }
  s.set = true;
  return OFFK_OK;
}

int offk_missing_weights(const offk_handle* h, char* buf, size_t buflen) {
  if (!h) return OFFK_ERR_INVALID;
  int missing = 0;
  for (const Slot& s : h->slots)
    if (!s.set) {
      if (missing == 0 && buf && buflen) snprintf(buf, buflen, "%s", s.key.c_str());
      ++missing;
    }
  return missing;
}

size_t offk_workspace_bytes(const offk_handle* h) { return h ? h->ws_bytes : 0; }

int offk_workspace_region(const offk_handle* h, const char* name, size_t* offset_bytes, size_t* nbytes) {
  if (!h || !name) return OFFK_ERR_INVALID;
  auto it = h->regions.find(name);
  if (it == h->regions.end()) { h->err = std::string("unknown workspace region: ") + name; return OFFK_ERR_INVALID; }
  if (offset_bytes) *offset_bytes = it->second.first;
  if (nbytes) *nbytes = it->second.second;
  return OFFK_OK;
}

int offk_set_profiling(offk_handle* h, int enable) {
  if (!h) return OFFK_ERR_INVALID;
  if (enable < 0 || enable > 2) return fail(h, OFFK_ERR_INVALID, "offk_set_profiling: 0 off, 1 per-stage events, 2 per-launch trace");
  h->profiling = enable;
  return OFFK_OK;
}

int offk_launch_times(offk_handle* h, char* names, size_t names_len, double* ms, int64_t* calls, int max_entries, int reset) {
  if (!h || max_entries < 0 || (max_entries > 0 && (!ms || !calls))) return fail(h, OFFK_ERR_INVALID, "offk_launch_times: bad argument");
  DeviceGuard guard(h->cfg.device);
  const int n = (int)h->tr_names.size();
  std::vector<double> sum(n, 0.0);
  std::vector<int64_t> cnt(n, 0);
  if (!h->tr_marks.empty()) HIP_TRY(h, hipEventSynchronize(h->tr_events[h->tr_marks.size() - 1]));
// ... 116 lines not shown
  TRY(check_parts(h, parts));
  for (int s = 0; s < kNumSites; ++s)
    for (int q = 0; q < parts[s].n_parts; ++q)
      if (reinterpret_cast<uintptr_t>(parts[s].data[q]) & (k.align - 1))
        return fail(h, OFFK_ERR_INVALID, f + ": " + k.noun + " feature map pointers must be " + std::to_string(k.align) + "-byte aligned (site " +
                                             kSites[s].name + ")");
  return OFFK_OK;
}

static int forward_parts_kind(offk_handle* h, void* stream, const FeatKind& k, int feat_dtype, const offk_feat_parts parts[OFFK_NUM_SITES],
                              float* out7, float* out14, float* out28, void* workspace, const char* fn) {
  if (!h || !parts || !out7 || !out14 || !workspace) return fail(h, OFFK_ERR_INVALID, std::string(fn) + ": null argument");
  TRY(check_feat(h, k, feat_dtype, parts, fn));
  return forward_parts(h, stream, parts, out7, out14, out28, workspace, feat_dtype, k.cl);
}

static int forward_kind(offk_handle* h, void* stream, const FeatKind& k, int feat_dtype, const void* const feats[OFFK_NUM_SITES], float* out7,
                        float* out14, float* out28, void* workspace, const char* fn) {
  if (!h || !feats) return fail(h, OFFK_ERR_INVALID, std::string(fn) + ": null argument");
  offk_feat_parts parts[kNumSites];
  TRY(whole_maps(h, feats, parts, fn));
  return forward_parts_kind(h, stream, k, feat_dtype, parts, out7, out14, out28, workspace, fn);
}

static int off_units_fused_kind(offk_handle* h, void* stream, const FeatKind& k, int feat_dtype, const void* const feats[OFFK_NUM_SITES],
                                void* workspace, const char* fn) {
  if (!h || !feats || !workspace) return fail(h, OFFK_ERR_INVALID, std::string(fn) + ": null argument");
  offk_feat_parts parts[kNumSites];
  TRY(whole_maps(h, feats, parts, fn));
  TRY(check_feat(h, k, feat_dtype, parts, fn));
  for (int s = 0; s < kNumSites; ++s) TRY(site_weights_ready(h, s, true, true));
  DeviceGuard guard(h->cfg.device);
  return run_off_units_fused(h, static_cast<hipStream_t>(stream), parts, workspace, nullptr, feat_dtype, k.cl);
}

int offk_forward_parts_typed(offk_handle* h, void* stream, int feat_dtype, const offk_feat_parts parts[OFFK_NUM_SITES], float* out7,
                             float* out14, float* out28, void* workspace) {
  if (feat_dtype == OFFK_FEAT_F32) return offk_forward_parts(h, stream, parts, out7, out14, out28, workspace);
  return forward_parts_kind(h, stream, kKind16, feat_dtype, parts, out7, out14, out28, workspace, "offk_forward_typed");
}

int offk_forward_typed(offk_handle* h, void* stream, int feat_dtype, const void* const feats[OFFK_NUM_SITES], float* out7,
                       float* out14, float* out28, void* workspace) {
  if (feat_dtype == OFFK_FEAT_F32)
    return offk_forward(h, stream, reinterpret_cast<const float* const*>(feats), out7, out14, out28, workspace);
  return forward_kind(h, stream, kKind16, feat_dtype, feats, out7, out14, out28, workspace, "offk_forward_typed");
}

int offk_off_units_fused_typed(offk_handle* h, void* stream, int feat_dtype, const void* const feats[OFFK_NUM_SITES], void* workspace) {
  if (feat_dtype == OFFK_FEAT_F32) return offk_off_units_fused(h, stream, reinterpret_cast<const float* const*>(feats), workspace);
  return off_units_fused_kind(h, stream, kKind16, feat_dtype, feats, workspace, "offk_off_units_fused_typed");
}

int offk_forward_parts_cl(offk_handle* h, void* stream, int feat_dtype, const offk_feat_parts parts[OFFK_NUM_SITES], float* out7,
                          float* out14, float* out28, void* workspace) {
  return forward_parts_kind(h, stream, kKindCl, feat_dtype, parts, out7, out14, out28, workspace, "offk_forward_cl");
}

int offk_forward_cl(offk_handle* h, void* stream, int feat_dtype, const void* const feats[OFFK_NUM_SITES], float* out7, float* out14,
                    float* out28, void* workspace) {
  return forward_kind(h, stream, kKindCl, feat_dtype, feats, out7, out14, out28, workspace, "offk_forward_cl");
}

int offk_off_units_fused_cl(offk_handle* h, void* stream, int feat_dtype, const void* const feats[OFFK_NUM_SITES], void* workspace) {
  return off_units_fused_kind(h, stream, kKindCl, feat_dtype, feats, workspace, "offk_off_units_fused_cl");
}

static int forward_parts(offk_handle* h, void* stream, const offk_feat_parts feats[OFFK_NUM_SITES], float* out7, float* out14,
                         float* out28, void* workspace, int feat_dtype, bool cl) {
  if (!h || !feats || !out7 || !out14 || !workspace) return fail(h, OFFK_ERR_INVALID, "offk_forward: null argument");
  TRY(check_parts(h, feats));
  TRY(check_ready(h));
  DeviceGuard guard(h->cfg.device);
  hipStream_t st = static_cast<hipStream_t>(stream);
  Fwd f;
  TRY(f.init(h, st, workspace, out7, out14, out28));
  TRY(f.units(feats, feat_dtype, cl));
  TRY(finalize_merged(h, st));
  TRY(finalize_derived(h, st));
  TRY(f.fusion28());
  TRY(f.fusion14());
  TRY(f.fusion7());
  return f.heads();
}

size_t offk_train_workspace_bytes(const offk_handle* h) { return h ? h->train_ws_bytes : 0; }

size_t offk_unit_grad_floats(const offk_handle* h) { return h ? h->grad_floats : 0; }

int offk_unit_grad_slot(const offk_handle* h, const char* key, size_t* offset_floats, size_t* count) {
  if (!h || !key) return OFFK_ERR_INVALID;
  std::string k(key);
  if (k.rfind("module.", 0) == 0) k = k.substr(7);
  auto it = h->grad_slots.find(k);
  if (it == h->grad_slots.end()) { h->err = "no unit gradient for key: " + k; return OFFK_ERR_INVALID; }
  if (offset_floats) *offset_floats = it->second.first;
  if (count) *count = it->second.second;
  return OFFK_OK;
}

int offk_off_units_train(offk_handle* h, void* stream, const float* const feats[OFFK_NUM_SITES], void* workspace,
                         uint64_t drop_seed, double drop_p) {
  return off_units_whole(h, stream, nullptr, OFFK_FEAT_F32, reinterpret_cast<MapPtrs>(feats), workspace, true, drop_seed, drop_p, "offk_off_units_train");
}

static int off_units_backward(offk_handle* h, void* stream, const float* const feats[OFFK_NUM_SITES],
                              const offk_grad_view gm[OFFK_NUM_SITES], void* workspace, uint64_t drop_seed, double drop_p,
                              float* grads, int accumulate, int feat_dtype, bool nhwc) {
  if (!h || !feats || !gm || !workspace || !grads) return fail(h, OFFK_ERR_INVALID, "offk_off_units_backward: null argument");
  DropCfg drop;
  TRY(make_drop(h, drop_seed, drop_p, &drop));
  for (int s = 0; s < kNumSites; ++s) {
    if (!feats[s] || !gm[s].data) return fail(h, OFFK_ERR_INVALID, "offk_off_units_backward: null feature map or gradient");
    if (gm[s].cstride < gm[s].coff + kUnitCh || (gm[s].cstride & 3) || (gm[s].coff & 3) || gm[s].coff < 0)
      return fail(h, OFFK_ERR_INVALID, "offk_off_units_backward: gradient view needs 16-byte aligned 160 channels inside cstride");
    TRY(site_weights_ready(h, s, false, true));
  }
  DeviceGuard guard(h->cfg.device);
  hipStream_t st = static_cast<hipStream_t>(stream);
  void* ws = workspace;
  const bool learned_dw = h->cfg.variant != OFFK_VARIANT_DIAG_SOBEL;
  auto reg = [&](const char* prefix, int s) { return region(h, ws, (std::string(prefix) + kSites[s].name).c_str()); };

  UbParams up;
  memset(&up, 0, sizeof(up));
  up.nsites = kNumSites; up.B = h->cfg.batch; up.L = h->cfg.length; up.tpix = kUbTpix;
  up.drop_thresh = drop.thresh; up.drop_scale = drop.scale; up.zeros = h->zero_page;
  int sblk = 0, tblk = 0;
  int nsblocks[kNumSites];
  for (int s = 0; s < kNumSites; ++s) {
    UbSite& u = up.s[s];
    u.G = reg("G_", s); u.D = reg("D_", s);
    u.dw = learned_dw ? (h->bnd_dw_w[s] ? h->bnd_dw_w[s] : h->dw_w[s]) : h->sobel_w;
    u.dw_ref = learned_dw && h->bnd_dw_w[s] != nullptr;
    u.gm = gm[s].data; u.gm_cs = gm[s].cstride; u.gm_coff = gm[s].coff;
    u.dG = reg("dG_", s); u.dD = reg("dD_", s);
    u.dw_part = learned_dw ? reg("dwp_", s) : nullptr;
    u.drop_base = drop_stream_base(drop.seed, s);
    u.H = kSites[s].H;
    ub_plan(u.H, &u.strips, &u.rows);
    u.tchunks = (u.H * u.H + kUbTpix - 1) / kUbTpix;
    u.s_begin = sblk; u.t_begin = tblk;
    nsblocks[s] = h->P * u.strips;
    sblk += nsblocks[s];
    tblk += h->cfg.batch * u.tchunks;
  }
  up.total_s = sblk; up.total_t = tblk;
  HIP_TRY(h, units_bwd_launch(up, st));

  WgParams wp;
  memset(&wp, 0, sizeof(wp));
  wp.nsites = kNumSites; wp.L = h->cfg.length; wp.P = h->P; wp.slice_mode = h->cfg.slice_mode; wp.kt_per_blk = h->wg_kpb;
  wp.precision = 0;
  wp.dbg = 0;
  wp.zeros = h->zero_page;
  WrParams rp;
  memset(&rp, 0, sizeof(rp));
  rp.nsites = kNumSites; rp.accumulate = accumulate ? 1 : 0;
  int blk = 0;
  for (int i = 0; i < kNumSites; ++i) {
    const int s = kPwOrder[i];
    WgSite& w = wp.s[i];
    w.xp[0] = feats[s]; w.cp[0] = kSites[s].C; w.nparts = 1;
    w.dG = reg("dG_", s); w.dD = reg("dD_", s); w.slab = reg("wgs_", s); w.bpart = reg("wgb_", s);
    w.C = kSites[s].C; w.HW = kSites[s].H * kSites[s].H;
    w.tpf = (w.HW + 31) / 32; w.kt_total = h->N * w.tpf;
// ... 342 lines not shown
```

### optical-flow-guided-feature-pytorch_amd/csrc/offk_internal.h

```cpp
#pragma once
#include <hip/hip_runtime.h>
#include <stddef.h>
#include <stdint.h>

namespace offk {

hipError_t lds_attr_once(const void* kernel, int bytes);

constexpr int OFFK_CONV_RELU_IN_ = 1, OFFK_CONV_RELU_PRE_ = 2, OFFK_CONV_RELU_POST_ = 4;
constexpr int kNumSites = 9;
constexpr int kGenCh = 128, kDownCh = 32, kUnitCh = 160;

struct ConvDesc {
  const float* x; int x_cs, x_coff;
  int n_img, H, W, Ci;
  const float* w;
  const float* bias;
  int Co, KH, KW, stride, pad;
  const float* res; int res_cs, res_coff;
  int flags;
  float* y; int y_cs, y_coff;
  int tile_cfg = -1, splitk = 0;
  float* partial = nullptr;
  size_t partial_floats = 0;
  int precision = 0;
  int co_limit = 0;
  int batch = 1;
  long long x_bstride = 0, w_bstride = 0, y_bstride = 0;
  int ngroups = 0;
  int g_batch[4] = {0, 0, 0, 0}, g_Ci[4] = {0, 0, 0, 0};
  long long g_x[4] = {0, 0, 0, 0}, g_w[4] = {0, 0, 0, 0}, g_y[4] = {0, 0, 0, 0};
  float* pool_part = nullptr;
  int pool_hw = 0;
};
void conv2d_auto_plan(long long M, int Co, int nkt, int* cfg_out, int* splitk_out, int precision);
hipError_t conv2d_launch(const ConvDesc& d, hipStream_t st, const char** why);
hipError_t pack_conv_weight_launch(const float* src, int Co, int Ci, int KH, int KW, float* dst, hipStream_t st);

struct ChainArgs {
  const float* x; int x_cs, x_coff;
  int Cin;
  int relu_in;
  const float* w1; const float* b1;
  const float* w2; const float* b2;
  const float* u2;
  const float* w3; const float* b3;
  int K3;
  const float* res; int res_cs, res_coff;
  float* y; int y_cs, y_coff;
  int n_img, relu_out;
  unsigned x_bytes;
  const void* w1p = nullptr; const void* w2p = nullptr; const void* w3p = nullptr;
  const void* wbp = nullptr; const float* bbr = nullptr;
#ifdef OFFK_CHAIN_TIMING
  unsigned long long* dbg;
#endif
};
hipError_t chain14_launch(const ChainArgs& a, hipStream_t st, const char** why);
bool chain14_split_supported(const ChainArgs& a);
hipError_t chain14_split_launch(const ChainArgs& a, hipStream_t st, const char** why);
hipError_t chain_wino_weight_launch(const float* w2_packed, float* U, hipStream_t st);

constexpr int kWinoPoints = 121, kWinoUnits4 = 400;
hipError_t wino_weight_launch(const float* w_packed, int Co, int Ci, int phases, float* U, hipStream_t st);
hipError_t wino_input_launch(const float* x, int x_cs, int x_coff, int n_img, int Ci, int phases, float* V, hipStream_t st);
hipError_t wino_output_launch(const float* M, int n_img, int Co, int phases, const float* bias, const float* res, int res_cs,
                              int res_coff, int flags, float* y, int y_cs, int y_coff, float* pool_part, hipStream_t st);
struct WinoGroup { int batch, kmul; long long v_off, u_off, m_off; };
int wino_groups(int phases, long long rows, int Ci, int Co, WinoGroup out[4]);
struct WinoGemmArgs {
  const float* x; const float* w; float* y;
  int M, Co;
  int ngroups, g_batch[4], g_K[4];
  long long g_x[4], g_w[4], g_y[4];
  int gm, gn, total_items;
  const void* w_planes = nullptr;
  long long x_bytes = 0, w_bytes = 0, y_bytes = 0;
  int epilogue = 0, x_rs = 0, x_coff = 0, y_rs = 0, y_coff = 0, relu = 0, pool_hw = 0;
  const float* bias = nullptr;
  float* pool_part = nullptr;
};
bool wino_gemm_supported(const WinoGemmArgs& a);
hipError_t wino_gemm_launch(const WinoGemmArgs& a, hipStream_t st);
bool wino_gemm_split_supported(const WinoGemmArgs& a);
hipError_t wino_gemm_split_launch(const WinoGemmArgs& a, hipStream_t st);
hipError_t wino_pack_split_launch(const float* U, void* img, int Co, int K, int nproblems, hipStream_t st);
struct WinoMidArgs {
  const float* M;
  const float* bias_in;
  int phases_in;
  float* x; int x_cs, x_coff;
  const float* w1;
  const float* b1;
  int Cin, Cmid, n_img;
  float* V;
  int nsplit = 0;
  const void* w1p = nullptr;
};
bool wino_mid_supported(int Cin, int Cmid, bool gemm, int phases_in);
hipError_t wino_mid_launch(const WinoMidArgs& a, hipStream_t st);
constexpr int kWino7Units = 225, kWino7Points = 64, kWino7Tiles = 9;
hipError_t wino7_weight_launch(const float* w_packed, int Co, int Ci, float* U, hipStream_t st);
hipError_t wino7_input_launch(const float* x, int x_cs, int x_coff, int n_img, int Ci, float* V, hipStream_t st);
hipError_t wino7_output_launch(const float* M, int n_img, int Co, const float* bias, int flags, float* y, int y_cs, int y_coff, hipStream_t st);
int wino7_groups(long long T, int Ci, int Co, WinoGroup out[4]);

struct PwSite {
  const float* xp[4];
  int cp[4];
  int nparts;
  const float* w;
  const float* w_down;
  const float* bias;
  const float* bias_down;
  float* G;
  float* D;
  int C, HW, M;
  int blk_begin;
};
struct PwParams {
  PwSite s[kNumSites];
  int nsites, total_blocks;
  int L, P, slice_mode, nhwc;
  const float* zeros;
#ifdef OFFK_TUNING_KNOBS
  int ablate;
#endif
};
int pw_blocks_for(int M);
hipError_t pw_reduce_launch(const PwParams& p, hipStream_t st);
constexpr int kFeatF32 = 0, kFeatBf16 = 1, kFeatF16 = 2;
constexpr int kFeatCl = 4;
bool pw_reduce_feat16_supported(const PwParams& p);
hipError_t pw_reduce_feat16_launch(const PwParams& p, int feat_dtype, hipStream_t st);
hipError_t pw_reduce_cl16_launch(const PwParams& p, int feat_dtype, hipStream_t st);

struct PtSite {
  const float* xp[4];
  int cp[4];
  int nparts;
  const float* w;
  const float* w_down;
  const float* wt;
  const float* wt16;
  const void* wt16s;
  const float* bias;
  const float* bias_down;
  float* D;
  float* M;
  int m_cs, m_coff;
  int C, HW;
  int chunks;
  int nrem;
  int rsh;
  int qpc;
  int blk_begin;
};
struct PtParams {
  PtSite s[kNumSites];
  int nsites, total_blocks;
  int B, L, P, slice_mode, tgroups;
  int f32split;
  int bdirect;
  const float* zeros;
#ifdef OFFK_PT_TIMING
  unsigned long long* dbg;
#endif
};
int pt_tgroups(int L);
hipError_t pw_tdiff_launch(const PtParams& p, hipStream_t st);
hipError_t pw_pack_direct16_launch(const float* w160, int C, float* out, hipStream_t st);
hipError_t pw_pack_split16_launch(const float* w160, int C, void* out, hipStream_t st);
hipError_t pw_tdiff_split_launch(const PtParams& p, hipStream_t st);
hipError_t pw_tdiff_feat16_launch(const PtParams& p, int feat_dtype, hipStream_t st);
hipError_t pw_tdiff_cl_launch(const PtParams& p, int feat_dtype, hipStream_t st);

struct StSite {
  const float* G;
  const float* D;
  const float* dw;
// ... 19 lines not shown
  float drop_scale;
  int taps4;
  const float* zeros;
};
void st_plan(int H, int* strips, int* rows);
void st_recips(int H, int* wrecip, int* twrecip);
int st_tchunks(int H);
int st_tchunks_flat(int H, int L);
hipError_t sobel_tdiff_launch(const StParams& p, int algo, hipStream_t st);

unsigned long long drop_stream_base(unsigned long long seed, int site);
struct UbSite {
  const float* G;
  const float* D;
  const float* dw;
  int dw_ref;
  const float* gm;
  int gm_cs, gm_coff;
  float* dG;
  float* dD;
  float* dw_part;
  unsigned long long drop_base;
  int H, strips, rows, tchunks, s_begin, t_begin;
};
struct UbParams {
  UbSite s[kNumSites];
  int nsites, total_s, total_t, B, L, tpix;
  unsigned drop_thresh;
  float drop_scale;
  const float* zeros;
};
hipError_t units_bwd_launch(const UbParams& p, hipStream_t st);

struct WgSite {
  const float* xp[4];
  int cp[4];
  int nparts;
  const float* dG;
  const float* dD;
  float* slab;
  float* bpart;
  int C, HW;
  int tpf;
  int kt_total;
  int ntiles;
  int nchunks;
  int blk_begin;
};
struct WgParams {
  WgSite s[kNumSites];
  int nsites, total_blocks, L, P, slice_mode, kt_per_blk;
  int precision;
  int dbg;
  const float* zeros;
};
hipError_t pw_wgrad_launch(const WgParams& p, hipStream_t st);
hipError_t pw_wgrad_feat16_launch(const WgParams& p, int feat_dtype, hipStream_t st);
hipError_t pw_wgrad_cl_launch(const WgParams& p, int feat_dtype, hipStream_t st);

struct WrSite {
  const float* slab; const float* bpart; const float* dw_part;
  float *gen_w, *gen_b, *down_w, *down_b, *dw_w, *dw_b;
  int C, cpad, nchunks, nsblocks;
};
struct WrParams {
  WrSite s[kNumSites];
  int nsites, accumulate;
};
hipError_t wgrad_reduce_launch(const WrParams& p, hipStream_t st);
hipError_t consensus_bwd_launch(const float* go, int B, int T, int C, float* gi, hipStream_t st);

hipError_t head_launch(const float* x, int x_cs, int x_coff, int n_img, int H, int W, int C, int maxpool, const float* fw,
                       const float* fb, int ncls, float* out, hipStream_t st, const char** why);
hipError_t pool_launch(const float* x, int x_cs, int x_coff, int n_img, int H, int W, int C, int maxpool, float* pooled,
                       hipStream_t st);
hipError_t fc_launch(const float* pooled, int n_img, int C, const float* fw, const float* fb, int ncls, float* out, hipStream_t st);
hipError_t maxpool_rows_launch(const float* x, int x_cs, int x_coff, int n_img, int H, int W, int C, float* part, hipStream_t st);
struct FcPooledJob { const float* part; int hw, tiles, C; const float* fw; const float* fb; float* out; };
struct FcPooledJobs { FcPooledJob job[3]; int njobs, n_img, ncls; };
hipError_t fc_pooled_multi_launch(const FcPooledJobs& j, hipStream_t st);
hipError_t fc_pooled_launch(const float* part, int hw, int tiles, int n_img, int C, const float* fw, const float* fb, int ncls, float* out,
                            hipStream_t st);
hipError_t vec_add_launch(const float* a, const float* b, float* o, int n, hipStream_t st);
hipError_t score_fusion_launch(const float* const* scores, const float* weights, int n, int videos, int crops, int classes,
                               float* fused, int* pred, hipStream_t st);
hipError_t consensus_launch(const float* x, int B, int T, int C, float* out, hipStream_t st);
hipError_t consensus_multi_launch(const float* const x[3], float* const out[3], int nheads, int B, int T, int C, hipStream_t st);
hipError_t nchw_to_nhwc_launch(const float* src, int n_img, int C, int HW, float* dst, hipStream_t st);
hipError_t nhwc_to_nchw_launch(const float* src, int cs, int coff, int n_img, int C, int HW, float* dst, hipStream_t st);
hipError_t repack_dw_launch(const float* w_c33, float* w_tap_c, hipStream_t st);

}
```

### optical-flow-guided-feature-pytorch_amd/csrc/wino_mid.hip

```cpp
#include <type_traits>

#include "offk_common.h"
#include "offk_internal.h"
#include "winograd_common.h"

namespace offk {

namespace {
typedef float f32x4 __attribute__((ext_vector_type(4)));
typedef unsigned u32x4 __attribute__((ext_vector_type(4)));

template <int C>
__device__ __forceinline__ int tile_off(int px, int c) { return px * (C * 4) + ((((c >> 2) ^ (px & 15))) << 4) + (c & 3) * 4; }

template <int LC> constexpr int kPlaneStride = (LC / 8) * 256;
template <int LC> constexpr int kPtStride = 3 * kPlaneStride<LC>;
template <int LC>
__device__ __forceinline__ int plane_off(int px, int c) {
  const int g = c >> 3;
  return (px >> 4) * kPtStride<LC> + g * 256 + ((((px & 15) ^ (2 * (g & 7)))) << 4) + (c & 7) * 2;
}
template <int LC>
__device__ __forceinline__ void store_planes(char* xt, int px, int c, float v) {
  const unsigned h = __float_as_uint(v) & 0xffff0000u;
  const float r = v - __uint_as_float(h);
  const unsigned m = __float_as_uint(r) & 0xffff0000u;
  const float l = r - __uint_as_float(m);
  char* d = xt + plane_off<LC>(px, c);
  *reinterpret_cast<unsigned short*>(d) = (unsigned short)(h >> 16);
  *reinterpret_cast<unsigned short*>(d + kPlaneStride<LC>) = (unsigned short)(m >> 16);
  *reinterpret_cast<unsigned short*>(d + 2 * kPlaneStride<LC>) = (unsigned short)(__float_as_uint(l) >> 16);
}

template <int NPH, int CY, int CX, int CIN, int G0 = 0, int G1 = CIN / 64, int LC = CIN, bool SPL = false>
__device__ __forceinline__ void mid_out_class(const WinoMidArgs& a, int img, int lane, char* xt, float* xg) {
  constexpr int NY = CY ? 5 : 6, NX = CX ? 5 : 6, OY = CY ? 3 : 4, OX = CX ? 3 : 4, oy = CY ? 4 : 0, ox = CX ? 4 : 0;
  const size_t pstride = (size_t)a.n_img * CIN;
#pragma unroll
  for (int g0 = G0; g0 < G1; g0 += 2) {
    float m[2][NY][NX];
#pragma unroll
    for (int u = 0; u < 2; ++u) {
      const float* mp = a.M + (size_t)img * CIN + (g0 + u) * 64 + lane;
#pragma unroll
      for (int j = 0; j < NX; ++j)
#pragma unroll
        for (int i = 0; i < NY; ++i) m[u][i][j] = mp[(size_t)wino_mindex<NPH, CY, CX>(i, j) * pstride];
    }
#pragma unroll
    for (int u = 0; u < 2; ++u) {
      const int c = (g0 + u) * 64 + lane;
      float s[OY][NX];
#pragma unroll
      for (int j = 0; j < NX; ++j) {
        float col[NY], sc[OY];
#pragma unroll
        for (int i = 0; i < NY; ++i) col[i] = m[u][i][j];
        wat(col, sc);
#pragma unroll
        for (int i = 0; i < OY; ++i) s[i][j] = sc[i];
      }
      const float bv = a.bias_in ? a.bias_in[c] : 0.f;
#pragma unroll
      for (int i = 0; i < OY; ++i) {
        float yv[OX];
        wat(s[i], yv);
#pragma unroll
        for (int j = 0; j < OX; ++j) {
          const int px = (oy + i) * 7 + ox + j;
          const float v = fmaxf(yv[j] + bv, 0.f);
          if constexpr (SPL) store_planes<LC>(xt, px, c - 64 * G0, v);
          else *reinterpret_cast<float*>(xt + tile_off<LC>(px, c - 64 * G0)) = v;
          if (xg) xg[((size_t)img * 49 + px) * a.x_cs + a.x_coff + c] = v;
        }
      }
    }
  }
}

template <int CY, int CX, int C, int CV>
__device__ __forceinline__ void mid_in_class(const WinoMidArgs& a, int img, int lane, int c_first, const char* ot) {
  constexpr int NY = CY ? 5 : 6, NX = CX ? 5 : 6;
  constexpr int oy = CY ? 4 : 0, ox = CX ? 4 : 0;
  const size_t pstride = (size_t)a.n_img * CV;
#pragma unroll
  for (int g = 0; g < C / 64; ++g) {
    const int c = g * 64 + lane;
    float t[NY][NX];
#pragma unroll
    for (int j = 0; j < NX; ++j)
#pragma unroll
      for (int i = 0; i < NY; ++i) {
        const int row = oy - 1 + i, col = ox - 1 + j;
        t[i][j] = row >= 0 && row < 7 && col >= 0 && col < 7 ? *reinterpret_cast<const float*>(ot + tile_off<C>(row * 7 + col, c)) : 0.f;
      }
#pragma unroll
    for (int j = 0; j < NX; ++j) {
      float d[NY], tc[NY];
#pragma unroll
      for (int i = 0; i < NY; ++i) d[i] = t[i][j];
      wbt(d, tc);
#pragma unroll
      for (int i = 0; i < NY; ++i) t[i][j] = tc[i];
    }
    float* vp = a.V + (size_t)img * CV + c_first + c;
#pragma unroll
    for (int i = 0; i < NY; ++i) {
      float v[NX];
      wbt(t[i], v);
#pragma unroll
      for (int j = 0; j < NX; ++j) vp[(size_t)wino_mindex<1, CY, CX>(i, j) * pstride] = v[j];
    }
  }
}
}

template <int CIN, int CMID, bool GEMM, int NPH, int NS, int KH = 1, bool SPL = false>
__global__ __launch_bounds__(256, (KH == 2 || SPL) ? 3 : 2) void wino_mid_kernel(WinoMidArgs a) {
  static_assert(!SPL || (GEMM && CIN / KH == 128), "split stage B: x tiles of 128 channels (48 KB of planes: three blocks per CU)");
  static_assert(CIN % 128 == 0 && CMID % (64 * NS) == 0 && (GEMM || (CIN == CMID && NS == 1)), "whole waves of channels");
  static_assert(KH == 1 || (KH == 2 && GEMM && CIN == 256), "k halves: the 256 -> 256 form");
  constexpr int CM = CMID / NS;
  constexpr int XC = CIN / KH;
  extern __shared__ __attribute__((aligned(16))) char lds[];
  const int img = blockIdx.x;
  const int c_first = (int)blockIdx.y * CM;
  const int tid = threadIdx.x, lane = tid & 63;
  const int wave = __builtin_amdgcn_readfirstlane(tid >> 6);

  float* const xg = blockIdx.y == 0 ? a.x : nullptr;
  auto zero_tail = [&]() {
    if constexpr (SPL) {
      for (int i = tid; i < kPtStride<XC> / 16; i += 256) reinterpret_cast<f32x4*>(lds + 3 * kPtStride<XC>)[i] = f32x4{0.f, 0.f, 0.f, 0.f};
      __syncthreads();
    } else {
      for (int i = tid; i < 15 * XC / 4; i += 256) reinterpret_cast<f32x4*>(lds + 49 * (XC * 4))[i] = f32x4{0.f, 0.f, 0.f, 0.f};
    }
  };
  auto stage_a = [&](auto half) {
    constexpr int H = decltype(half)::value;
    constexpr int G0 = KH == 2 ? 2 * H : 0, G1 = KH == 2 ? 2 * H + 2 : CIN / 64;
    switch (wave) {
      case 0: mid_out_class<NPH, 0, 0, CIN, G0, G1, XC, SPL>(a, img, lane, lds, xg); break;
      case 1: mid_out_class<NPH, 0, 1, CIN, G0, G1, XC, SPL>(a, img, lane, lds, xg); break;
      case 2: mid_out_class<NPH, 1, 0, CIN, G0, G1, XC, SPL>(a, img, lane, lds, xg); break;
      default: mid_out_class<NPH, 1, 1, CIN, G0, G1, XC, SPL>(a, img, lane, lds, xg); break;
    }
  };
  if constexpr (GEMM) zero_tail();
  stage_a(std::integral_constant<int, 0>{});
  __syncthreads();

  if constexpr (GEMM) {
    constexpr int CT = CM / 64, PT = 4, KS = CIN / 16, KSH = KS / KH;
    const int li = lane & 15, kq = lane >> 4;
    const __amdgpu_buffer_rsrc_t wrs = __builtin_amdgcn_make_buffer_rsrc(const_cast<float*>(a.w1), 0, CMID * CIN * 4, 0x00020000);
    const int wvoff = ((c_first + wave * (CM / 4) + li) * CIN + 4 * kq) * 4;
    auto w_load = [&](f32x4 (&w)[CT], const int s) {
// ... 59 lines not shown
            for (int ct = 0; ct < CT; ++ct) acs[pt][ct] = mfs(acs[pt][ct], wq[t & 1][ct][1], x[1]);
#pragma unroll
            for (int ct = 0; ct < CT; ++ct) acs[pt][ct] = mfs(acs[pt][ct], wq[t & 1][ct][1], x[0]);
#pragma unroll
            for (int ct = 0; ct < CT; ++ct) acs[pt][ct] = mfs(acs[pt][ct], wq[t & 1][ct][0], x[1]);
            __builtin_amdgcn_sched_barrier(0);
          }
        }
      }
    };
    auto stage_b = [&](const int s0) {
      if constexpr (SPL) { stage_b_split(s0 / 2); return; }
      f32x4 wq[3][CT], xv[2][PT];
      w_load(wq[0], s0);
      if (KSH > 1) w_load(wq[1], s0 + 1);
      x_load(xv[0], 0);
#pragma unroll
      for (int s = 0; s < KSH; ++s) {
        if (s + 2 < KSH) w_load(wq[(s + 2) % 3], s0 + s + 2);
        if (s + 1 < KSH) x_load(xv[(s + 1) & 1], s + 1);
        __builtin_amdgcn_sched_barrier(0);
        const f32x4 (&w)[CT] = wq[s % 3];
        const f32x4 (&x)[PT] = xv[s & 1];
#pragma unroll
        for (int pt = 0; pt < PT; ++pt)
#pragma unroll
          for (int ct = 0; ct < CT; ++ct) acc[pt][ct] = __builtin_amdgcn_mfma_f32_16x16x4f32(w[ct].x, x[pt].x, acc[pt][ct], 0, 0, 0);
#pragma unroll
        for (int pt = 0; pt < PT; ++pt)
#pragma unroll
          for (int ct = 0; ct < CT; ++ct) acc[pt][ct] = __builtin_amdgcn_mfma_f32_16x16x4f32(w[ct].y, x[pt].y, acc[pt][ct], 0, 0, 0);
#pragma unroll
        for (int pt = 0; pt < PT; ++pt)
#pragma unroll
          for (int ct = 0; ct < CT; ++ct) acc[pt][ct] = __builtin_amdgcn_mfma_f32_16x16x4f32(w[ct].z, x[pt].z, acc[pt][ct], 0, 0, 0);
#pragma unroll
        for (int pt = 0; pt < PT; ++pt)
#pragma unroll
          for (int ct = 0; ct < CT; ++ct) acc[pt][ct] = __builtin_amdgcn_mfma_f32_16x16x4f32(w[ct].w, x[pt].w, acc[pt][ct], 0, 0, 0);
        __builtin_amdgcn_sched_barrier(0);
      }
    };
    stage_b(0);
    if constexpr (KH == 2) {
      __syncthreads();
      zero_tail();
      stage_a(std::integral_constant<int, 1>{});
      __syncthreads();
      stage_b(KSH);
    }
    __syncthreads();
#pragma unroll
    for (int ct = 0; ct < CT; ++ct) {
      const int ch = wave * (CM / 4) + 16 * ct + 4 * kq;
      const f32x4 bb = *reinterpret_cast<const f32x4*>(a.b1 + c_first + ch);
#pragma unroll
      for (int pt = 0; pt < PT; ++pt) {
        const int px = 16 * pt + li;
        f32x4 v = acc[pt][ct] + bb;
        if constexpr (SPL) v = (acc[pt][ct] + acs[pt][ct]) + bb;
        if (px < 49)
          *reinterpret_cast<f32x4*>(lds + tile_off<CM>(px, ch)) = f32x4{fmaxf(v.x, 0.f), fmaxf(v.y, 0.f), fmaxf(v.z, 0.f), fmaxf(v.w, 0.f)};
      }
    }
    __syncthreads();
  }

  switch (wave) {
    case 0: mid_in_class<0, 0, CM, CMID>(a, img, lane, c_first, lds); break;
    case 1: mid_in_class<0, 1, CM, CMID>(a, img, lane, c_first, lds); break;
    case 2: mid_in_class<1, 0, CM, CMID>(a, img, lane, c_first, lds); break;
    default: mid_in_class<1, 1, CM, CMID>(a, img, lane, c_first, lds); break;
  }
}

bool wino_mid_supported(int Cin, int Cmid, bool gemm, int phases_in) {
  if (gemm) return (Cin == 128 && Cmid == 128 && (phases_in == 4 || phases_in == 1)) || (Cin == 256 && Cmid == 256 && phases_in == 1);
  return Cin == Cmid && (Cin == 128 || Cin == 256) && phases_in == 1;
}

hipError_t wino_mid_launch(const WinoMidArgs& a, hipStream_t st) {
  const bool gemm = a.w1 != nullptr;
  if (!wino_mid_supported(a.Cin, a.Cmid, gemm, a.phases_in) || a.n_img < 1 || !a.M || !a.V || (gemm && !a.b1) ||
      (a.x && (a.x_cs % 4 || a.x_coff % 4)))
    return hipErrorInvalidValue;
#define OFFK_MID_LAUNCH_KH(CI, CM, G, PH, NSP, KHV)                                                                \
  {                                                                                                                \
    constexpr int kLds = 64 * (CI / KHV > CM / NSP ? CI / KHV : CM / NSP) * 4;                                     \
    hipError_t e = lds_attr_once(reinterpret_cast<const void*>(wino_mid_kernel<CI, CM, G, PH, NSP, KHV>), kLds);   \
    if (e != hipSuccess) return e;                                                                                 \
    hipLaunchKernelGGL((wino_mid_kernel<CI, CM, G, PH, NSP, KHV>), dim3(a.n_img, NSP), dim3(256), kLds, st, a);    \
  }
#define OFFK_MID_LAUNCH_SPL(CI, CM, PH, KHV)                                                                                  \
  {                                                                                                                           \
    constexpr int kLds = 4 * kPtStride<CI / KHV>;                                                                             \
    static_assert(kLds >= 64 * (CM / 2) * 4, "t tile behind the planes");                                                     \
    hipError_t e = lds_attr_once(reinterpret_cast<const void*>(wino_mid_kernel<CI, CM, true, PH, 2, KHV, true>), kLds);       \
    if (e != hipSuccess) return e;                                                                                            \
    hipLaunchKernelGGL((wino_mid_kernel<CI, CM, true, PH, 2, KHV, true>), dim3(a.n_img, 2), dim3(256), kLds, st, a);          \
    return hipGetLastError();                                                                                                 \
  }
  if (gemm && a.w1p && a.nsplit <= 0) {
    if (a.Cin == 128 && a.phases_in == 4) OFFK_MID_LAUNCH_SPL(128, 128, 4, 1)
    else if (a.Cin == 128) OFFK_MID_LAUNCH_SPL(128, 128, 1, 1)
    else OFFK_MID_LAUNCH_SPL(256, 256, 1, 2)
  }
#undef OFFK_MID_LAUNCH_SPL
#define OFFK_MID_LAUNCH(CI, CM, G, PH, NSP) OFFK_MID_LAUNCH_KH(CI, CM, G, PH, NSP, 1)
#ifndef OFFK_MID_NS256
#define OFFK_MID_NS256 22
#endif
  const int ns = a.nsplit > 0 ? a.nsplit : (gemm && a.Cin == 128 ? 2 : OFFK_MID_NS256);
  if (gemm && a.Cin == 128 && a.phases_in == 4) { if (ns == 2) OFFK_MID_LAUNCH(128, 128, true, 4, 2) else OFFK_MID_LAUNCH(128, 128, true, 4, 1) }
  else if (gemm && a.Cin == 128) { if (ns == 2) OFFK_MID_LAUNCH(128, 128, true, 1, 2) else OFFK_MID_LAUNCH(128, 128, true, 1, 1) }
  else if (gemm) { if (ns == 4) OFFK_MID_LAUNCH(256, 256, true, 1, 4) else if (ns == 2) OFFK_MID_LAUNCH(256, 256, true, 1, 2) else if (ns == 22) OFFK_MID_LAUNCH_KH(256, 256, true, 1, 2, 2) else OFFK_MID_LAUNCH(256, 256, true, 1, 1) }
  else if (a.Cin == 128) OFFK_MID_LAUNCH(128, 128, false, 1, 1)
  else OFFK_MID_LAUNCH(256, 256, false, 1, 1)
#undef OFFK_MID_LAUNCH
#undef OFFK_MID_LAUNCH_KH
  return hipGetLastError();
}

}
```

### optical-flow-guided-feature-pytorch_amd/csrc/winograd.hip

```cpp
#include "offk_common.h"
#include "offk_internal.h"
#include "winograd_common.h"

namespace offk {

namespace {
template <int NPH, int CY, int CX>
__device__ __forceinline__ void wino_input_tile(const float* __restrict__ xi, int x_cs, int R, int img, int Ci, int pa, int pb,
                                                unsigned c, float* __restrict__ V) {
  constexpr int NY = CY ? 5 : 6, NX = CX ? 5 : 6, W = NPH == 1 ? 7 : 14, STEP = NPH == 1 ? 1 : 2;
  constexpr int oy = CY ? 4 : 0, ox = CX ? 4 : 0;
  const unsigned c4 = c * 4u;
  float t[NY][NX];
#pragma unroll
  for (int j = 0; j < NX; ++j)
#pragma unroll
    for (int i = 0; i < NY; ++i) {
      const int row = oy - 1 + i, col = ox - 1 + j;
      t[i][j] = row >= 0 && row < 7 && col >= 0 && col < 7
                    ? *reinterpret_cast<const float*>(reinterpret_cast<const char*>(xi + (size_t)((STEP * row + pa) * W + STEP * col + pb) * x_cs) + c4)
                    : 0.f;
    }
#pragma unroll
  for (int j = 0; j < NX; ++j) {
    float d[NY], tc[NY];
#pragma unroll
    for (int i = 0; i < NY; ++i) d[i] = t[i][j];
    wbt(d, tc);
#pragma unroll
    for (int i = 0; i < NY; ++i) t[i][j] = tc[i];
  }
  const int K = NPH * Ci;
#pragma unroll
  for (int i = 0; i < NY; ++i) {
    float v[NX];
    wbt(t[i], v);
#pragma unroll
    for (int j = 0; j < NX; ++j) {
      if constexpr (NPH == 1) {
        *reinterpret_cast<float*>(reinterpret_cast<char*>(V + ((size_t)wino_mindex<1, CY, CX>(i, j) * R + img) * K) + c4) = v[j];
      } else {
        WinoPlace pl;
        if (wino_place4<CY, CX>(i, j, pa, pb, pl))
          __builtin_nontemporal_store(v[j], reinterpret_cast<float*>(reinterpret_cast<char*>(V + ((size_t)pl.base_ci * R + ((size_t)pl.idx * R + img) * pl.kmul + pl.slot) * Ci) + c4));
      }
    }
  }
}
}

template <int NPH>
__global__ __launch_bounds__(256) void wino_input_kernel(const float* __restrict__ x, int x_cs, int x_coff, int n_img, int Ci,
                                                         float* __restrict__ V) {
  constexpr int W = NPH == 1 ? 7 : 14;
  const int cw = (Ci + 63) >> 6;
  const int wid = __builtin_amdgcn_readfirstlane((int)((blockIdx.x * 256u + threadIdx.x) >> 6));
  if (wid >= 4 * n_img * NPH * cw) return;
  const int img = wid / (4 * NPH * cw), r0 = wid - img * (4 * NPH * cw);
  const int cls = r0 / (NPH * cw), r1 = r0 - cls * (NPH * cw), ph = r1 / cw, pa = ph >> 1, pb = ph & 1;
  const unsigned c = (unsigned)(r1 - ph * cw) * 64u + (threadIdx.x & 63u);
  if (c >= (unsigned)Ci) return;
  const float* xi = x + (size_t)img * W * W * x_cs + x_coff;
  switch (cls) {
    case 0: wino_input_tile<NPH, 0, 0>(xi, x_cs, n_img, img, Ci, pa, pb, c, V); break;
    case 1: wino_input_tile<NPH, 0, 1>(xi, x_cs, n_img, img, Ci, pa, pb, c, V); break;
    case 2: wino_input_tile<NPH, 1, 0>(xi, x_cs, n_img, img, Ci, pa, pb, c, V); break;
    default: wino_input_tile<NPH, 1, 1>(xi, x_cs, n_img, img, Ci, pa, pb, c, V); break;
  }
}

struct WinoOutArgs {
  const float* M;
  const float* bias;
  const float* res; int res_cs, res_coff;
  float* y; int y_cs, y_coff;
  float* pool_part;
  int n_img, Co, flags;
};
namespace {
template <int NPH, int CY, int CX>
__device__ __forceinline__ void wino_output_tile(const WinoOutArgs& a, int img, unsigned c) {
  constexpr int NY = CY ? 5 : 6, NX = CX ? 5 : 6, OY = CY ? 3 : 4, OX = CX ? 3 : 4, oy = CY ? 4 : 0, ox = CX ? 4 : 0;
  const float* mp = a.M + (size_t)img * a.Co + c;
  const size_t pstride = (size_t)a.n_img * a.Co;
  float s[OY][NX];
#pragma unroll
  for (int j = 0; j < NX; ++j) {
    float m[NY], sc[OY];
#pragma unroll
    for (int i = 0; i < NY; ++i) m[i] = mp[(size_t)wino_mindex<NPH, CY, CX>(i, j) * pstride];
    wat(m, sc);
#pragma unroll
    for (int i = 0; i < OY; ++i) s[i][j] = sc[i];
  }
  const float bv = a.bias ? a.bias[c] : 0.f;
  const bool relu_pre = a.flags & OFFK_CONV_RELU_PRE_, relu_post = a.flags & OFFK_CONV_RELU_POST_;
  float psum = 0.f;
#pragma unroll
  for (int i = 0; i < OY; ++i) {
    float yv[OX];
    wat(s[i], yv);
#pragma unroll
    for (int j = 0; j < OX; ++j) {
      const size_t pix = (size_t)img * 49 + (oy + i) * 7 + ox + j;
      float v = yv[j] + bv;
      if (relu_pre) v = fmaxf(v, 0.f);
      if (a.res) v += a.res[pix * a.res_cs + a.res_coff + c];
      if (relu_post) v = fmaxf(v, 0.f);
      a.y[pix * a.y_cs + a.y_coff + c] = v;
      psum += v;
    }
  }
  if (a.pool_part) a.pool_part[((size_t)img * 4 + 2 * CY + CX) * a.Co + c] = psum;
}
}
template <int NPH>
__global__ __launch_bounds__(256) void wino_output_kernel(WinoOutArgs a) {
  const int cw = (a.Co + 63) >> 6;
  const int wid = __builtin_amdgcn_readfirstlane((int)((blockIdx.x * 256u + threadIdx.x) >> 6));
  if (wid >= 4 * a.n_img * cw) return;
  const int cls = wid / (a.n_img * cw), r0 = wid - cls * (a.n_img * cw), img = r0 / cw;
  const unsigned c = (unsigned)(r0 - img * cw) * 64u + (threadIdx.x & 63u);
  if (c >= (unsigned)a.Co) return;
  switch (cls) {
    case 0: wino_output_tile<NPH, 0, 0>(a, img, c); break;
    case 1: wino_output_tile<NPH, 0, 1>(a, img, c); break;
    case 2: wino_output_tile<NPH, 1, 0>(a, img, c); break;
    default: wino_output_tile<NPH, 1, 1>(a, img, c); break;
  }
}

namespace {
template <int NPH, int CY, int CX>
__device__ __forceinline__ void wino_weight_tile(const float (&g)[3][3], int Co, int co, int Ci, int ci, int pa, int pb, int kk,
                                                 float* __restrict__ U) {
  constexpr int NY = CY ? 5 : 6, NX = CX ? 5 : 6;
  float t[NY][3];
#pragma unroll
  for (int v = 0; v < 3; ++v) {
    float gc[3], u[NY];
#pragma unroll
    for (int i = 0; i < 3; ++i) gc[i] = g[i][v];
    wg(gc, u);
#pragma unroll
    for (int i = 0; i < NY; ++i) t[i][v] = u[i];
  }
  const int K = NPH * Ci;
#pragma unroll
  for (int i = 0; i < NY; ++i) {
    float u[NX];
    wg(t[i], u);
#pragma unroll
    for (int j = 0; j < NX; ++j) {
      if constexpr (NPH == 1) {
        U[((size_t)wino_mindex<1, CY, CX>(i, j) * Co + co) * K + kk] = u[j];
      } else {
        WinoPlace pl;
        if (wino_place4<CY, CX>(i, j, pa, pb, pl))
          U[((size_t)pl.base_ci * Co + ((size_t)pl.idx * Co + co) * pl.kmul + pl.slot) * Ci + ci] = u[j];
      }
    }
  }
}
}
template <int NPH>
__global__ __launch_bounds__(256) void wino_weight_kernel(const float* __restrict__ w, int Co, int Ci, float* __restrict__ U) {
  constexpr int KS = NPH == 1 ? 3 : 5, STEP = NPH == 1 ? 1 : 2;
  const int K = NPH * Ci;
  const long long gid = (long long)blockIdx.x * 256 + threadIdx.x;
  if (gid >= (long long)Co * K) return;
  const int co = (int)(gid / K), kk = (int)(gid - (long long)co * K);
  const int ph = kk / Ci, ci = kk - ph * Ci, pa = ph >> 1, pb = ph & 1;
  const float* wp = w + ((size_t)(co * (Ci / 32) + ci / 32) * (KS * KS)) * 32 + (ci & 31);
  float g[3][3];
#pragma unroll
  for (int i = 0; i < 3; ++i)
#pragma unroll
    for (int j = 0; j < 3; ++j) {
      const int kh = STEP * i + pa, kw = STEP * j + pb;
      g[i][j] = kh < KS && kw < KS ? wp[(size_t)(kh * KS + kw) * 32] : 0.f;
    }
  wino_weight_tile<NPH, 0, 0>(g, Co, co, Ci, ci, pa, pb, kk, U);
  wino_weight_tile<NPH, 0, 1>(g, Co, co, Ci, ci, pa, pb, kk, U);
  wino_weight_tile<NPH, 1, 0>(g, Co, co, Ci, ci, pa, pb, kk, U);
  wino_weight_tile<NPH, 1, 1>(g, Co, co, Ci, ci, pa, pb, kk, U);
}

int wino_groups(int phases, long long rows, int Ci, int Co, WinoGroup out[4]) {
  if (phases == 1) { out[0] = WinoGroup{kWinoPoints, 1, 0, 0, 0}; return 1; }
  const int batch[4] = {81, 18, 18, 4}, kmul[4] = {4, 2, 2, 1}, base[4] = {0, 324, 360, 396}, first[4] = {0, 81, 99, 117};
  for (int g = 0; g < 4; ++g)
    out[g] = WinoGroup{batch[g], kmul[g], (long long)base[g] * rows * Ci, (long long)base[g] * Co * Ci, (long long)first[g] * rows * Co};
  return 4;
}

hipError_t wino_weight_launch(const float* w_packed, int Co, int Ci, int phases, float* U, hipStream_t st) {
  const long long n = (long long)Co * Ci * phases;
  if (phases == 4) hipLaunchKernelGGL(wino_weight_kernel<4>, dim3((unsigned)((n + 255) / 256)), dim3(256), 0, st, w_packed, Co, Ci, U);
  else hipLaunchKernelGGL(wino_weight_kernel<1>, dim3((unsigned)((n + 255) / 256)), dim3(256), 0, st, w_packed, Co, Ci, U);
  return hipGetLastError();
}

hipError_t wino_input_launch(const float* x, int x_cs, int x_coff, int n_img, int Ci, int phases, float* V, hipStream_t st) {
  const long long waves = (long long)4 * n_img * phases * ((Ci + 63) / 64);
  if (phases == 4) hipLaunchKernelGGL(wino_input_kernel<4>, dim3((unsigned)((waves + 3) / 4)), dim3(256), 0, st, x, x_cs, x_coff, n_img, Ci, V);
  else hipLaunchKernelGGL(wino_input_kernel<1>, dim3((unsigned)((waves + 3) / 4)), dim3(256), 0, st, x, x_cs, x_coff, n_img, Ci, V);
  return hipGetLastError();
}

hipError_t wino_output_launch(const float* M, int n_img, int Co, int phases, const float* bias, const float* res, int res_cs,
                              int res_coff, int flags, float* y, int y_cs, int y_coff, float* pool_part, hipStream_t st) {
  WinoOutArgs a;
  a.M = M; a.bias = bias; a.res = res; a.res_cs = res_cs; a.res_coff = res_coff;
  a.y = y; a.y_cs = y_cs; a.y_coff = y_coff; a.pool_part = pool_part;
  a.n_img = n_img; a.Co = Co; a.flags = flags;
  const long long waves = (long long)4 * n_img * ((Co + 63) / 64);
  if (phases == 4) hipLaunchKernelGGL(wino_output_kernel<4>, dim3((unsigned)((waves + 3) / 4)), dim3(256), 0, st, a);
  else hipLaunchKernelGGL(wino_output_kernel<1>, dim3((unsigned)((waves + 3) / 4)), dim3(256), 0, st, a);
  return hipGetLastError();
}

}
```

### optical-flow-guided-feature-pytorch_amd/runtime.py

```python
import collections
import ctypes

import numpy as np
import torch

from . import _lib, spec


def _ptr(t):
    return ctypes.c_void_p(t.data_ptr()) if t is not None else ctypes.c_void_p(0)


def _stream(device=None):
    return ctypes.c_void_p(torch.cuda.current_stream(device).cuda_stream)


def _check_dev(t, name, device):
    if not (torch.is_tensor(t) and t.is_cuda and t.dtype == torch.float32 and t.is_contiguous()):
        raise ValueError("%s must be a contiguous fp32 CUDA/HIP tensor" % name)
    if t.device != device:
        raise ValueError("%s lives on %s, handle on %s" % (name, t.device, device))


def _given(t, shape, name, device, dtype=torch.float32):
# ... 126 lines not shown
        self.batch, self.length, self.variant = int(batch), int(length), int(variant)
        self.slice_mode, self.consensus, self.num_classes = int(slice_mode), bool(consensus), int(num_classes)
        self.feat_layout = int(feat_layout)
        self.precision = _lib.PRECISIONS[precision] if isinstance(precision, str) else int(precision)
        self.N = self.batch * self.length
        self.P = self.batch * (self.length - 1)
        cfg = _lib.OffkConfig(self.batch, self.length, self.variant, self.slice_mode, int(self.consensus),
                              self.num_classes, self.feat_layout, self.device.index or 0, self.precision)
        h = ctypes.c_void_p()
        _lib.check(self.lib.offk_create(ctypes.byref(cfg), ctypes.byref(h)))
        self._h = h
        self._ws = None
        self.training = bool(training)

    def __del__(self):
        h = getattr(self, "_h", None)
        if h:
            self.lib.offk_destroy(h)
            self._h = None

    def set_weight(self, key, value):
        if torch.is_tensor(value):
            t = value.detach().to(dtype=torch.float32).contiguous()
            shape = tuple(t.shape)
            ptr, keep = ctypes.c_void_p(t.data_ptr()), t
        else:
            a = np.ascontiguousarray(value, dtype=np.float32)
            shape = a.shape
            ptr, keep = ctypes.c_void_p(a.ctypes.data), a
        arr = (ctypes.c_int64 * len(shape))(*shape)
        _lib.check(self.lib.offk_set_weight(self._h, key.encode(), ptr, arr, len(shape)), self._h)
        del keep

    def bind_weight(self, key, tensor):
        _check_dev(tensor, key, self.device)
        kk = key[7:] if key.startswith("module.") else key
        want = spec.weight_shapes(self.variant).get(kk)
        if want is not None and tuple(tensor.shape) != tuple(want):
            raise ValueError("%s has shape %s, the reference's is %s" % (key, tuple(tensor.shape), tuple(want)))
        shape = (ctypes.c_int64 * tensor.dim())(*tensor.shape)
        _lib.check(self.lib.offk_bind_weight(self._h, key.encode(), ctypes.c_void_p(tensor.data_ptr()), shape, tensor.dim()), self._h)

    def load_state_dict(self, state_dict, strict=True):
        want = spec.weight_shapes(self.variant)
        seen = set()
        for k, v in state_dict.items():
            kk = k[7:] if k.startswith("module.") else k
            if kk in want:
                self.set_weight(kk, v)
                seen.add(kk)
        missing = [k for k in want if k not in seen]
        if strict and missing:
            raise KeyError("missing OFF weights: %s" % ", ".join(missing[:5]))
        return missing

    def missing_weights(self):
        buf = ctypes.create_string_buffer(256)
        n = self.lib.offk_missing_weights(self._h, buf, 256)
        return n, buf.value.decode()

    @property
    def workspace_bytes(self):
        if self.training:
            return int(self.lib.offk_train_workspace_bytes(self._h))
        return int(self.lib.offk_workspace_bytes(self._h))

    @property
    def workspace(self):
        if self._ws is None:
            self._ws = torch.empty(self.workspace_bytes, dtype=torch.uint8, device=self.device)
        return self._ws

    def set_workspace(self, t):
        if not (torch.is_tensor(t) and t.is_cuda and t.dtype == torch.uint8 and t.is_contiguous()):
            raise ValueError("the workspace must be a contiguous uint8 CUDA/HIP tensor")
        if t.device != self.device:
            raise ValueError("the workspace lives on %s, handle on %s" % (t.device, self.device))
        if t.numel() < self.workspace_bytes:
            raise ValueError("the workspace holds %d bytes, the handle needs %d" % (t.numel(), self.workspace_bytes))
        self._ws = t

    def region(self, name, channels):
        off, nb = ctypes.c_size_t(), ctypes.c_size_t()
        _lib.check(self.lib.offk_workspace_region(self._h, name.encode(), ctypes.byref(off), ctypes.byref(nb)), self._h)
        flat = self.workspace[off.value:off.value + nb.value].view(torch.float32)
        return flat.view(-1, channels)

    def out_rows(self):
        return self.batch if self.consensus else self.P

    def _route(self, feats, side):
        return feat_route(feats, self.batch, self.length, self.feat_layout, self.precision, side)

    def takes_channels_last(self, feats):
        return (self.feat_layout == 0 and len(feats) == spec.NUM_SITES
                and _all_channels_last(feats, self.batch, self.length, "infer", self.precision == _lib.PRECISION_F32SPLIT))

    def train_takes_channels_last(self, feats):
        return train_feat_layout(feats, self.batch, self.length) == "cl"

    def _call(self, op, r, *args):
        head = (self._h, _stream(self.device)) + (() if r.route == "plain" else (r.fdt,))
        _lib.check(getattr(self.lib, _ENTRIES[op][r.route][0])(*(head + args)), self._h)

    def _units_call(self, op, feats, *tail):
        r = self._route(feats, _SIDES[op])
        self._call(op, r, self._feat_array(feats, _ENTRIES[op][r.route][1]), _ptr(self.workspace), *tail)

    def _feat_array(self, feats, check=_check_dev):
        if len(feats) != spec.NUM_SITES:
            raise ValueError("need nine feature maps")
        shapes = spec.feature_shapes(self.batch, self.length)
        for i, (f, s) in enumerate(zip(feats, shapes)):
            check(f, "feats[%d]" % i, self.device)
            want = s if self.feat_layout == 0 or check is _check_dev_cl else (s[0], s[2], s[3], s[1])
            if tuple(f.shape) != tuple(want):
                raise ValueError("feats[%d] has shape %s, expected %s" % (i, tuple(f.shape), tuple(want)))
        return (ctypes.c_void_p * spec.NUM_SITES)(*[f.data_ptr() for f in feats])

    def _parts_array(self, feats, check=_check_dev):
        shapes = spec.feature_shapes(self.batch, self.length)
        arr = (_lib.OffkFeatParts * spec.NUM_SITES)()
        for i, (f, s) in enumerate(zip(feats, shapes)):
            parts = [f] if torch.is_tensor(f) else list(f)
            if not 1 <= len(parts) <= 4:
                raise ValueError("feats[%d]: 1..4 channel groups" % i)
            arr[i].n_parts = len(parts)
            for q, t in enumerate(parts):
                check(t, "feats[%d][%d]" % (i, q), self.device)
                c = t.shape[1] if self.feat_layout == 0 else t.shape[3]
                want = (s[0], c, s[2], s[3]) if self.feat_layout == 0 else (s[0], s[2], s[3], c)
                if tuple(t.shape) != want:
                    raise ValueError("feats[%d][%d] has shape %s, expected %s" % (i, q, tuple(t.shape), want))
                arr[i].channels[q] = c
                arr[i].data[q] = t.data_ptr()
        return arr

    def _outs(self, out, want28):
        shape = (self.out_rows(), self.num_classes)
        if out is None:
            out7 = torch.empty(shape, dtype=torch.float32, device=self.device)
            return out7, torch.empty_like(out7), torch.empty_like(out7) if want28 else None
        out7, out14, out28 = out
        return (_given(out7, shape, "out7", self.device), _given(out14, shape, "out14", self.device),
                _given(out28, shape, "out28", self.device) if out28 is not None else None)

    def forward(self, feats, want28=True, out=None):
        r = self._route(feats, "infer")
        if r.route == "cl":
            return self._forward_cl(feats, want28, **({} if out is None else {"out": out}))
        return self._forward(feats, want28, out, r)

    def _forward(self, feats, want28, out, r):
        op = "forward_parts" if r.parts else "forward"
        arr = (self._parts_array if r.parts else self._feat_array)(feats, _ENTRIES[op][r.route][1])
        out7, out14, out28 = self._outs(out, want28)
        self._call(op, r, arr, _ptr(out7), _ptr(out14), _ptr(out28), _ptr(self.workspace))
        return out7, out14, out28

    def _forward_cl(self, feats, want28, out=None):
        return self._forward(feats, want28, out, self._route(feats, "infer"))

    def forward_into(self, feat_array, out7, out14, out28):
        _lib.check(self.lib.offk_forward(self._h, _stream(self.device), feat_array, _ptr(out7), _ptr(out14), _ptr(out28),
                                         _ptr(self.workspace)), self._h)

# ... 290 lines not shown
```

Before: 23420 clips/s.

## Pool before the merged 7x7 conv and fold it into a composed head

At the 7x7 stage the channel sums are pooled directly in the winograd mid and output transforms. The merged 1x1 conv is folded algebraically into the FC weights, giving a derived composed head. This skips materialising the 1024-channel sum_7 map during forward. sum_7 is now computed lazily only when a caller asks for that region, which adds a deferred-state flag and a dirty-tracking path for the composed weights.

```diff
diff --git a/include/offk.h b/include/offk.h
--- a/include/offk.h
+++ b/include/offk.h
@@ -92,6 +92,8 @@
                           float* out7, float* out14, float* out28, void* workspace);
 
 int offk_workspace_region(const offk_handle* h, const char* name, size_t* offset_bytes, size_t* nbytes);
+
+int offk_stage_tensors(offk_handle* h, void* stream, void* workspace);
 
 #define OFFK_NUM_STAGES 6
 int offk_set_profiling(offk_handle* h, int enable);
diff --git a/optical-flow-guided-feature-pytorch_amd/_lib.py b/optical-flow-guided-feature-pytorch_amd/_lib.py
--- a/optical-flow-guided-feature-pytorch_amd/_lib.py
+++ b/optical-flow-guided-feature-pytorch_amd/_lib.py
@@ -53,6 +53,7 @@
     "offk_forward_cl": (_I, [_P, _P, _I, _c.POINTER(_P), _F, _F, _F, _P]),
     "offk_forward_parts_cl": (_I, [_P, _P, _I, _c.POINTER(OffkFeatParts), _F, _F, _F, _P]),
     "offk_workspace_region": (_I, [_P, _c.c_char_p, _c.POINTER(_c.c_size_t), _c.POINTER(_c.c_size_t)]),
+    "offk_stage_tensors": (_I, [_P, _P, _P]),
     "offk_set_profiling": (_I, [_P, _I]),
     "offk_stage_times": (_I, [_P, _c.POINTER(_c.c_double), _c.POINTER(_c.c_int64), _I]),
     "offk_launch_times": (_I, [_P, _c.c_char_p, _c.c_size_t, _c.POINTER(_c.c_double), _c.POINTER(_c.c_int64), _I, _I]),
diff --git a/optical-flow-guided-feature-pytorch_amd/csrc/heads.hip b/optical-flow-guided-feature-pytorch_amd/csrc/heads.hip
--- a/optical-flow-guided-feature-pytorch_amd/csrc/heads.hip
+++ b/optical-flow-guided-feature-pytorch_amd/csrc/heads.hip
@@ -315,6 +315,24 @@
   return hipGetLastError();
 }
 
+__global__ __launch_bounds__(256) void head_compose_kernel(const float* __restrict__ fw, const float* __restrict__ fb, const float* __restrict__ wm,
+                                                           const float* __restrict__ bm, int Cm, int K, float* __restrict__ w_out,
+                                                           float* __restrict__ b_out) {
+  const int cls = blockIdx.y, k = blockIdx.x * 256 + threadIdx.x;
+  if (k > K) return;
+  const float* f = fw + (size_t)cls * Cm;
+  double acc = 0.0;
+  for (int j = 0; j < Cm; ++j) acc += (double)f[j] * (double)(k < K ? wm[(size_t)j * K + k] : bm[j]);
+  if (k < K) w_out[(size_t)cls * K + k] = (float)acc;
+  else b_out[cls] = (float)(acc + (double)fb[cls]);
+}
+hipError_t head_compose_launch(const float* fw, const float* fb, int ncls, const float* wm, const float* bm, int Cm, int K, float* w_out,
+                               float* b_out, hipStream_t st) {
+  if (ncls <= 0 || Cm <= 0 || K <= 0) return hipErrorInvalidValue;
+  hipLaunchKernelGGL(head_compose_kernel, dim3((K + 1 + 255) / 256, ncls), dim3(256), 0, st, fw, fb, wm, bm, Cm, K, w_out, b_out);
+  return hipGetLastError();
+}
+
 __global__ void consensus_kernel(const float* __restrict__ x, int T, int C, float* __restrict__ out) {
   const int b = blockIdx.x;
   for (int c = threadIdx.x; c < C; c += blockDim.x) {
diff --git a/optical-flow-guided-feature-pytorch_amd/csrc/offk_api.hip b/optical-flow-guided-feature-pytorch_amd/csrc/offk_api.hip
--- a/optical-flow-guided-feature-pytorch_amd/csrc/offk_api.hip
+++ b/optical-flow-guided-feature-pytorch_amd/csrc/offk_api.hip
@@ -123,6 +123,7 @@
   float* u2 = nullptr;
   float* planes = nullptr;
   float* gemm_planes = nullptr;
+  float* head = nullptr;
 };
 constexpr int kNumDerived = kNumConvs + 3;
 constexpr int merged_slot(int m) { return kNumConvs + m; }
@@ -189,6 +190,8 @@
   int conv_cfg[kNumConvs];
   int conv_splitk[kNumConvs];
   size_t splitk_floats = 0;
+  bool pool_first7 = false;
+  bool sum7_pending = false;
   bool fold_pool = true;
   std::vector<void*> allocs;
   std::map<std::string, std::pair<size_t, size_t>> regions;
@@ -308,6 +311,7 @@
     add_region(h, "wino_v", std::max((size_t)kWinoUnits4 * P * 1056, (size_t)kWino7Tiles * P * kWino7Units * 320));
     add_region(h, "wino_m", (size_t)kWinoPoints * P * 512);
     add_region(h, "poolpart_14t", (size_t)4 * P * 512);
+    if (h->pool_first7) add_region(h, "poolpart_7t", (size_t)4 * P * 512);
   }
   h->splitk_floats = (size_t)std::min<size_t>(64, std::max<size_t>(8, 1536 / P)) * P * 196 * 64;
   add_region(h, "splitk", h->splitk_floats);
@@ -651,7 +655,8 @@
   DK_U_F54,
   DK_CHAIN_U2,
   DK_PLANES,
-  DK_U_PLANES
+  DK_U_PLANES,
+  DK_HEAD_COMPOSED
 };
 DerivedKind u_kind(const ConvSpec& c) { return c.K == 7 ? DK_U_F54 : c.K == 5 ? DK_U_POLY : DK_U_F43; }
 int u_units(DerivedKind k) { return k == DK_U_F54 ? kWino7Units : k == DK_U_POLY ? kWinoUnits4 : kWinoPoints; }
@@ -662,7 +667,7 @@
 }
 size_t plane_floats(size_t elems) { return (elems * 3 + 1) / 2; }
 
-enum { ON_7X7 = 1, ON_SPLIT_GEMM = 2, ON_CHAIN_WINO = 4, ON_SPLIT_CHAIN = 8, ON_SPLIT_MID = 16 };
+enum { ON_7X7 = 1, ON_SPLIT_GEMM = 2, ON_CHAIN_WINO = 4, ON_SPLIT_CHAIN = 8, ON_SPLIT_MID = 16, ON_POOL_FIRST7 = 32 };
 struct DerivedRow {
   int slot;
   DerivedKind kind;
@@ -673,7 +678,7 @@
 };
 bool derived_exists(const offk_handle* h, const DerivedRow& r) {
   const int on = h->wino_7x7 * ON_7X7 | h->split_gemm * ON_SPLIT_GEMM | h->chain_wino * ON_CHAIN_WINO | (h->chain && h->split_chain) * ON_SPLIT_CHAIN |
-                 (h->wino_mid && h->split_mid) * ON_SPLIT_MID;
+                 (h->wino_mid && h->split_mid) * ON_SPLIT_MID | h->pool_first7 * ON_POOL_FIRST7;
   const bool shape = r.kind != DK_U_PLANES || (kConvs[r.slot].Co % 64 == 0 && kConvs[r.slot].Ci >= 64);
   return h->winograd && !(r.needs & ~on) && shape && !(h->split_gemm_skip & r.skip_bit);
 }
@@ -692,7 +697,8 @@
     {CB_28A, DK_PLANES, &Derived::planes, ON_SPLIT_CHAIN},
     {C1_28B, DK_PLANES, &Derived::planes, ON_SPLIT_CHAIN}, {C2_28B, DK_PLANES, &Derived::planes, ON_SPLIT_CHAIN}, {C3_28B, DK_PLANES, &Derived::planes, ON_SPLIT_CHAIN},
     {C1_28C, DK_PLANES, &Derived::planes, ON_SPLIT_CHAIN}, {C2_28C, DK_PLANES, &Derived::planes, ON_SPLIT_CHAIN}, {C3_28C, DK_PLANES, &Derived::planes, ON_SPLIT_CHAIN},
-    {C1_14A, DK_PLANES, &Derived::planes, ON_SPLIT_MID}, {C1_7, DK_PLANES, &Derived::planes, ON_SPLIT_MID}};
+    {C1_14A, DK_PLANES, &Derived::planes, ON_SPLIT_MID}, {C1_7, DK_PLANES, &Derived::planes, ON_SPLIT_MID},
+    {merged_slot(2), DK_HEAD_COMPOSED, &Derived::head, ON_POOL_FIRST7}};
 
 struct Matrix { const float* w; int Co, K; };
 Matrix slot_matrix(const offk_handle* h, int slot) {
@@ -706,6 +712,7 @@
     case DK_CHAIN_U2: return (size_t)16 * 64 * 64;
     case DK_PLANES: { const Matrix m = slot_matrix(h, r.slot); return plane_floats((size_t)m.Co * (r.alloc_K ? r.alloc_K : m.K)); }
     case DK_U_PLANES: return plane_floats(u_elems(kConvs[r.slot]));
+    case DK_HEAD_COMPOSED: return (size_t)h->cfg.num_classes * (slot_matrix(h, r.slot).K + 1);
   }
   return 0;
 }
@@ -730,6 +737,12 @@
         HIP_TRY(h, wino_pack_split_launch(d.u + grp[g].u_off, reinterpret_cast<char*>(d.u_planes) + grp[g].u_off * 6, c.Co, grp[g].kmul * c.Ci, grp[g].batch, st));
       break;
     }
+    case DK_HEAD_COMPOSED: {
+      const Matrix m = slot_matrix(h, r.slot);
+      HIP_TRY(h, head_compose_launch(h->fc_w[0], h->fc_b[0], h->cfg.num_classes, m.w, h->merged_b[r.slot - kNumConvs], m.Co, m.K, d.head,
+                                     d.head + (size_t)h->cfg.num_classes * m.K, st));
+      break;
+    }
   }
   return OFFK_OK;
 }
@@ -791,13 +804,13 @@
   float *out7, *out14, *out28;
   float *l7, *l14, *l28;
   FcPooledJobs fcj{};
-  bool wino, w7, mid, w5, chained, fold, fold14t;
+  bool wino, w7, mid, w5, chained, fold, fold14t, pool7;
 
   float* reg(const char* name) const { return region(h, ws, name); }
 
-  int init(offk_handle* handle, hipStream_t st, void* workspace, float* o7, float* o14, float* o28) {
+  int init(offk_handle* handle, hipStream_t st, void* workspace, float* o7, float* o14, float* o28, bool stage_only = false) {
     h = handle; s = st; ws = workspace; n = h->P; out7 = o7; out14 = o14; out28 = o28;
-    if (h->profiling == 1) {
+    if (h->profiling == 1 && !stage_only) {
       const size_t per = OFFK_NUM_STAGES + 1;
       if ((h->ev_used + 1) * per > h->events.size() && h->events.size() < 4096 * per) {
         for (size_t i = 0; i < per; ++i) {
@@ -816,6 +829,7 @@
     auto generic = [](int cfg) { return cfg != 6 && cfg != 7 && cfg != 10; };
     fold = h->fold_pool && generic(h->conv_cfg[C3_14B]) && generic(h->merged_cfg[2]);
     fold14t = wino && h->fold_pool;
+    pool7 = h->pool_first7 && mid && fold14t && h->derived[merged_slot(2)].head;
     F14 = reg("fusion_14"); F7 = reg("fusion_7"); splitk = reg("splitk");
     wino_V = wino ? reg("wino_v") : nullptr;
     wino_M = wino ? reg("wino_m") : nullptr;
@@ -881,11 +895,11 @@
     if (e != hipSuccess) return fail(h, why ? OFFK_ERR_INVALID : OFFK_ERR_HIP, std::string(c.key) + " (winograd): " + (why ? why : hipGetErrorString(e)));
     return OFFK_OK;
   }
-  int wino_out(ConvId id, const float* res, int res_cs, int res_coff, int flags, float* y, int y_cs, int y_coff, float* pool_t) {
+  int wino_out(ConvId id, const float* res, int res_cs, int res_coff, int flags, float* y, int y_cs, int y_coff, float* pool_t, int pool_cs = 0) {
     const ConvSpec& c = kConvs[id];
     TRY(trace_mark(h, s, c.key, " [winograd: output transform]"));
     if (u_kind(c) == DK_U_F54) HIP_TRY(h, wino7_output_launch(wino_M, n, c.Co, h->conv_b[id], flags, y, y_cs, y_coff, s));
-    else HIP_TRY(h, wino_output_launch(wino_M, n, c.Co, wino_phases(c), h->conv_b[id], res, res_cs, res_coff, flags, y, y_cs, y_coff, pool_t, s));
+    else HIP_TRY(h, wino_output_launch(wino_M, n, c.Co, wino_phases(c), h->conv_b[id], res, res_cs, res_coff, flags, y, y_cs, y_coff, pool_t, s, pool_cs, 0));
     return OFFK_OK;
   }
   int wino_conv(ConvId id, View x, const float* res, int res_cs, int res_coff, int flags, float* y, int y_cs, int y_coff, float* pool_t) {
@@ -893,22 +907,24 @@
     TRY(wino_mm(id));
     return wino_out(id, res, res_cs, res_coff, flags, y, y_cs, y_coff, pool_t);
   }
-  int wino_between(ConvId a, ConvId c1, float* xa, int xa_cs, int xa_coff, const char* name) {
+  int wino_between(ConvId a, ConvId c1, float* xa, int xa_cs, int xa_coff, const char* name, float* pool_t = nullptr) {
     const bool has = c1 != kNumConvs;
-    const WinoMidArgs m = wino_mid_args(wino_M, h->conv_b[a], wino_phases(kConvs[a]), n, kConvs[a].Co, xa, xa_cs, xa_coff, has ? h->conv_w[c1] : nullptr,
+    WinoMidArgs m = wino_mid_args(wino_M, h->conv_b[a], wino_phases(kConvs[a]), n, kConvs[a].Co, xa, xa_cs, xa_coff, has ? h->conv_w[c1] : nullptr,
                                         has ? h->conv_b[c1] : nullptr, kConvs[has ? c1 : a].Co, wino_V, has ? h->derived[c1].planes : nullptr);
+    m.pool_part = pool_t; m.pool_cs = xa_cs; m.pool_coff = xa_coff;
     TRY(trace_mark(h, s, name));
     HIP_TRY(h, wino_mid_launch(m, s));
     return OFFK_OK;
   }
-  int conv_t_c1_c2(ConvId ct, bool wino_t, int H, View F, ConvId c1, ConvId c2, float* xx, int cs, float* t, const char* between) {
+  int conv_t_c1_c2(ConvId ct, bool wino_t, int H, View F, ConvId c1, ConvId c2, float* xx, int cs, float* t, const char* between,
+                   float* pool_t = nullptr) {
     const int half = cs / 2;
     if (wino_t && mid) {
       TRY(wino_in(ct, F));
       TRY(wino_mm(ct));
-      TRY(wino_between(ct, c1, xx, cs, half, between));
+      TRY(wino_between(ct, c1, xx, cs, half, between, pool_t));
       TRY(wino_mm(c2));
-      return wino_out(c2, nullptr, 0, 0, RP, xx, cs, 0, nullptr);
+      return wino_out(c2, nullptr, 0, 0, RP, xx, cs, 0, pool_t, pool_t ? cs : 0);
     }
     if (wino_t) TRY(wino_conv(ct, F, nullptr, 0, 0, RP, xx, cs, half, nullptr));
     else TRY(conv(ct, H, F, nullptr, 0, 0, RP, xx, cs, half));
@@ -1008,13 +1024,22 @@
 
   int fusion7() {
     float *xv = reg("xv_7"), *v1 = reg("v1_7"), *s7 = reg("sum_7");
+    float* pp7t = pool7 ? reg("poolpart_7t") : nullptr;
     TRY(conv_t_c1_c2(C_T7, wino, 7, View{F7, 832, 0}, C1_7, C2_7, xv, 512, v1,
-                     "motion_conv_trans out + motion_conv1_trans + motion_conv2_trans in [winograd: between]"));
+                     "motion_conv_trans out + motion_conv1_trans + motion_conv2_trans in [winograd: between]", pp7t));
+    if (pool7) {
+      const float* wc = h->derived[merged_slot(2)].head;
+      fcj.job[fcj.njobs++] = FcPooledJob{pp7t, 49, 1, 512, wc, wc + (size_t)h->cfg.num_classes * 512, l7};
+      h->sum7_pending = true;
+      if (ev) HIP_TRY(h, hipEventRecord(ev[5], s));
+      return OFFK_OK;
+    }
     float* pp7 = fold ? reg("poolpart_7") : nullptr;
-    TRY(conv_merged(2, 7, View{xv, 512, 0}, 0, s7, 1024, 0, pp7));
+    TRY(merged7());
     if (ev) HIP_TRY(h, hipEventRecord(ev[5], s));
     return head(0, l7, pp7, 0, s7, 1024, 0, 7, 0, "pooled_7");
   }
+  int merged7() { return conv_merged(2, 7, View{reg("xv_7"), 512, 0}, 0, reg("sum_7"), 1024, 0, fold ? reg("poolpart_7") : nullptr); }
 
   int heads() {
     if (fcj.njobs > 0) {
@@ -1141,6 +1166,11 @@
   { const char* e = getenv("OFFK_SPLIT_GEMM_SKIP"); if (e) h->split_gemm_skip = atoi(e); }
 #endif
   h->chain_wino = h->winograd && h->chain && path_switch("OFFK_CHAIN_WINO");
+  {
+    int gate = 96;
+    const bool on = path_switch("OFFK_POOL_FIRST_7", &gate);
+    h->pool_first7 = on && h->winograd && h->wino_mid && h->fold_pool && h->P >= gate;
+  }
   for (const DerivedRow& r : kDerived)
     if (rc == OFFK_OK && derived_exists(h, r)) rc = dev_alloc(h, &(h->derived[r.slot].*r.image), derived_floats(h, r));
   if (rc != OFFK_OK) {
@@ -1235,6 +1265,8 @@
   }
   if (s.kind == SK_CONV_W || s.kind == SK_CONV_B) h->merged_dirty = true;
   if (s.kind == SK_CONV_W) h->derived_dirty = true;
+  if (h->derived[merged_slot(2)].head && ((s.kind == SK_CONV_B && (i == C3_7 || i == CB_7)) || ((s.kind == SK_FC_W || s.kind == SK_FC_B) && i == 0)))
+    h->derived_dirty = true;
   if (s.kind == SK_GEN_W || s.kind == SK_DOWN_W) h->pw_dirty = true;
   return rc;
 }
@@ -1517,6 +1549,23 @@
   TRY(f.fusion14());
   TRY(f.fusion7());
   return f.heads();
+}
+
+int offk_stage_tensors(offk_handle* h, void* stream, void* workspace) {
+  if (!h || !workspace) return fail(h, OFFK_ERR_INVALID, "offk_stage_tensors: null argument");
+  if (!h->sum7_pending) return OFFK_OK;
+  DeviceGuard guard(h->cfg.device);
+  hipStream_t st = static_cast<hipStream_t>(stream);
+  Fwd f;
+  TRY(f.init(h, st, workspace, nullptr, nullptr, nullptr, true));
+  TRY(finalize_merged(h, st));
+  TRY(finalize_derived(h, st));
+  const int prof = h->profiling;
+  h->profiling = 0;
+  const int rc = f.merged7();
+  h->profiling = prof;
+  if (rc == OFFK_OK) h->sum7_pending = false;
+  return rc;
 }
 
 size_t offk_train_workspace_bytes(const offk_handle* h) { return h ? h->train_ws_bytes : 0; }
diff --git a/optical-flow-guided-feature-pytorch_amd/csrc/offk_internal.h b/optical-flow-guided-feature-pytorch_amd/csrc/offk_internal.h
--- a/optical-flow-guided-feature-pytorch_amd/csrc/offk_internal.h
+++ b/optical-flow-guided-feature-pytorch_amd/csrc/offk_internal.h
@@ -65,7 +65,8 @@
 hipError_t wino_weight_launch(const float* w_packed, int Co, int Ci, int phases, float* U, hipStream_t st);
 hipError_t wino_input_launch(const float* x, int x_cs, int x_coff, int n_img, int Ci, int phases, float* V, hipStream_t st);
 hipError_t wino_output_launch(const float* M, int n_img, int Co, int phases, const float* bias, const float* res, int res_cs,
-                              int res_coff, int flags, float* y, int y_cs, int y_coff, float* pool_part, hipStream_t st);
+                              int res_coff, int flags, float* y, int y_cs, int y_coff, float* pool_part, hipStream_t st, int pool_cs = 0,
+                              int pool_coff = 0);
 struct WinoGroup { int batch, kmul; long long v_off, u_off, m_off; };
 int wino_groups(int phases, long long rows, int Ci, int Co, WinoGroup out[4]);
 struct WinoGemmArgs {
@@ -96,6 +97,8 @@
   float* V;
   int nsplit = 0;
   const void* w1p = nullptr;
+  float* pool_part = nullptr;
+  int pool_cs = 0, pool_coff = 0;
 };
 bool wino_mid_supported(int Cin, int Cmid, bool gemm, int phases_in);
 hipError_t wino_mid_launch(const WinoMidArgs& a, hipStream_t st);
@@ -281,6 +284,8 @@
 hipError_t fc_pooled_launch(const float* part, int hw, int tiles, int n_img, int C, const float* fw, const float* fb, int ncls, float* out,
                             hipStream_t st);
 hipError_t vec_add_launch(const float* a, const float* b, float* o, int n, hipStream_t st);
+hipError_t head_compose_launch(const float* fw, const float* fb, int ncls, const float* wm, const float* bm, int Cm, int K, float* w_out,
+                               float* b_out, hipStream_t st);
 hipError_t score_fusion_launch(const float* const* scores, const float* weights, int n, int videos, int crops, int classes,
                                float* fused, int* pred, hipStream_t st);
 hipError_t consensus_launch(const float* x, int B, int T, int C, float* out, hipStream_t st);
diff --git a/optical-flow-guided-feature-pytorch_amd/csrc/wino_mid.hip b/optical-flow-guided-feature-pytorch_amd/csrc/wino_mid.hip
--- a/optical-flow-guided-feature-pytorch_amd/csrc/wino_mid.hip
+++ b/optical-flow-guided-feature-pytorch_amd/csrc/wino_mid.hip
@@ -61,6 +61,7 @@
         for (int i = 0; i < OY; ++i) s[i][j] = sc[i];
       }
       const float bv = a.bias_in ? a.bias_in[c] : 0.f;
+      float psum = 0.f;
 #pragma unroll
       for (int i = 0; i < OY; ++i) {
         float yv[OX];
@@ -72,8 +73,10 @@
           if constexpr (SPL) store_planes<LC>(xt, px, c - 64 * G0, v);
           else *reinterpret_cast<float*>(xt + tile_off<LC>(px, c - 64 * G0)) = v;
           if (xg) xg[((size_t)img * 49 + px) * a.x_cs + a.x_coff + c] = v;
+          psum += v;
         }
       }
+      if (xg && a.pool_part) a.pool_part[((size_t)img * 4 + 2 * CY + CX) * a.pool_cs + a.pool_coff + c] = psum;
     }
   }
 }
@@ -299,7 +302,7 @@
 hipError_t wino_mid_launch(const WinoMidArgs& a, hipStream_t st) {
   const bool gemm = a.w1 != nullptr;
   if (!wino_mid_supported(a.Cin, a.Cmid, gemm, a.phases_in) || a.n_img < 1 || !a.M || !a.V || (gemm && !a.b1) ||
-      (a.x && (a.x_cs % 4 || a.x_coff % 4)))
+      (a.x && (a.x_cs % 4 || a.x_coff % 4)) || (a.pool_part && (!a.x || a.pool_coff < 0 || a.pool_coff + a.Cin > a.pool_cs)))
     return hipErrorInvalidValue;
 #define OFFK_MID_LAUNCH_KH(CI, CM, G, PH, NSP, KHV)                                                                \
   {                                                                                                                \
diff --git a/optical-flow-guided-feature-pytorch_amd/csrc/winograd.hip b/optical-flow-guided-feature-pytorch_amd/csrc/winograd.hip
--- a/optical-flow-guided-feature-pytorch_amd/csrc/winograd.hip
+++ b/optical-flow-guided-feature-pytorch_amd/csrc/winograd.hip
@@ -75,6 +75,7 @@
   const float* res; int res_cs, res_coff;
   float* y; int y_cs, y_coff;
   float* pool_part;
+  int pool_cs, pool_coff;
   int n_img, Co, flags;
 };
 namespace {
@@ -111,7 +112,7 @@
       psum += v;
     }
   }
-  if (a.pool_part) a.pool_part[((size_t)img * 4 + 2 * CY + CX) * a.Co + c] = psum;
+  if (a.pool_part) a.pool_part[((size_t)img * 4 + 2 * CY + CX) * a.pool_cs + a.pool_coff + c] = psum;
 }
 }
 template <int NPH>
@@ -209,10 +210,12 @@
 }
 
 hipError_t wino_output_launch(const float* M, int n_img, int Co, int phases, const float* bias, const float* res, int res_cs,
-                              int res_coff, int flags, float* y, int y_cs, int y_coff, float* pool_part, hipStream_t st) {
+                              int res_coff, int flags, float* y, int y_cs, int y_coff, float* pool_part, hipStream_t st, int pool_cs, int pool_coff) {
+  if (pool_part && pool_cs > 0 && (pool_coff < 0 || pool_coff + Co > pool_cs)) return hipErrorInvalidValue;
   WinoOutArgs a;
   a.M = M; a.bias = bias; a.res = res; a.res_cs = res_cs; a.res_coff = res_coff;
   a.y = y; a.y_cs = y_cs; a.y_coff = y_coff; a.pool_part = pool_part;
+  a.pool_cs = pool_cs > 0 ? pool_cs : Co; a.pool_coff = pool_cs > 0 ? pool_coff : 0;
   a.n_img = n_img; a.Co = Co; a.flags = flags;
   const long long waves = (long long)4 * n_img * ((Co + 63) / 64);
   if (phases == 4) hipLaunchKernelGGL(wino_output_kernel<4>, dim3((unsigned)((waves + 3) / 4)), dim3(256), 0, st, a);
diff --git a/optical-flow-guided-feature-pytorch_amd/runtime.py b/optical-flow-guided-feature-pytorch_amd/runtime.py
--- a/optical-flow-guided-feature-pytorch_amd/runtime.py
+++ b/optical-flow-guided-feature-pytorch_amd/runtime.py
@@ -232,6 +232,8 @@
 
     def region(self, name, channels):
         off, nb = ctypes.c_size_t(), ctypes.c_size_t()
+        if name == "sum_7":
+            _lib.check(self.lib.offk_stage_tensors(self._h, _stream(self.device), _ptr(self.workspace)), self._h)
         _lib.check(self.lib.offk_workspace_region(self._h, name.encode(), ctypes.byref(off), ctypes.byref(nb)), self._h)
         flat = self.workspace[off.value:off.value + nb.value].view(torch.float32)
         return flat.view(-1, channels)
```

Result: faster. 24430 clips/s (median of 6 runs) (+4.3%).
